# ColinWine/Multi-modal-Multi-label-Facial-Action-Unit-Detection-with-Transformer

Measured on NVIDIA B200. Metric: AVFormer hot-path clips/sec (forward), higher is better.
Workload: dtype bf16

## Files before the change

multi-modal-multi-label-facial-action-unit-detection-with-transformer_b200/csrc/avf_fused_helpers.cuh:

```cuda
#pragma once
#include "avf_common.cuh"

namespace avf {
namespace fused {

#ifdef AVF_FUSED_PROF
static __device__ unsigned long long g_prof[64];
struct Prof {
  long long t0;
  bool on;
  unsigned acc[64];
  __device__ __forceinline__ void start(bool enable) {
    on = enable;
    for (int i = 0; i < 64; ++i) acc[i] = 0;
    t0 = clock64();
  }
  __device__ __forceinline__ void mark(int idx) {
    if (on) {
      const long long t1 = clock64();
      acc[idx] += unsigned(t1 - t0);
      t0 = t1;
    }
  }
  __device__ __forceinline__ void count(int idx) { if (on) acc[idx] += 1; }
  __device__ __forceinline__ void flush(int lo, int hi) {
    if (on) for (int i = lo; i < hi; ++i) g_prof[i] += acc[i];
  }
};
#else
struct Prof {
  __device__ __forceinline__ void start(bool) {}
  __device__ __forceinline__ void mark(int) {}
  __device__ __forceinline__ void count(int) {}
  __device__ __forceinline__ void flush(int, int) {}
};
#endif

__device__ __forceinline__ void bar_sync(int id, int count) { asm volatile("bar.sync %0, %1;" ::"r"(id), "r"(count) : "memory"); }
__device__ __forceinline__ uint32_t cvt_bf16x2(float lo, float hi) {
  uint32_t r;
  asm("cvt.rn.bf16x2.f32 %0, %1, %2;" : "=r"(r) : "f"(hi), "f"(lo));
  return r;
}
__device__ __forceinline__ uint32_t ex2_bf16x2(uint32_t x) {
  uint32_t r;
  asm("ex2.approx.ftz.bf16x2 %0, %1;" : "=r"(r) : "r"(x));
  return r;
}
__device__ __forceinline__ uint32_t tanh_bf16x2(uint32_t x) {
  uint32_t r;
  asm("tanh.approx.bf16x2 %0, %1;" : "=r"(r) : "r"(x));
  return r;
}
__device__ __forceinline__ uint32_t mul_bf16x2(uint32_t a, uint32_t b) {
  uint32_t r;
  asm("mul.rn.bf16x2 %0, %1, %2;" : "=r"(r) : "r"(a), "r"(b));
  return r;
}
__device__ __forceinline__ uint32_t fma_bf16x2(uint32_t a, uint32_t b, uint32_t c) {
  uint32_t r;
  asm("fma.rn.bf16x2 %0, %1, %2, %3;" : "=r"(r) : "r"(a), "r"(b), "r"(c));
  return r;
}
__device__ __forceinline__ uint32_t gelu_bf16x2(uint32_t x) {
  constexpr uint32_t C0 = 0x3F4C3F4Cu;
  constexpr uint32_t C1 = 0x3D123D12u;
  constexpr uint32_t HALF = 0x3F003F00u;
  const uint32_t x2 = mul_bf16x2(x, x);
  const uint32_t u = mul_bf16x2(x, fma_bf16x2(x2, C1, C0));
  const uint32_t hx = mul_bf16x2(x, HALF);
  return fma_bf16x2(hx, tanh_bf16x2(u), hx);
}
__device__ __forceinline__ uint64_t f2_pack(float lo, float hi) {
  uint64_t r;
  asm("mov.b64 %0, {%1, %2};" : "=l"(r) : "f"(lo), "f"(hi));
  return r;
}
__device__ __forceinline__ void f2_unpack(uint64_t v, float& lo, float& hi) { asm("mov.b64 {%0, %1}, %2;" : "=f"(lo), "=f"(hi) : "l"(v)); }
__device__ __forceinline__ uint64_t f2_add(uint64_t a, uint64_t b) {
  uint64_t r;
  asm("add.rn.f32x2 %0, %1, %2;" : "=l"(r) : "l"(a), "l"(b));
  return r;
}
__device__ __forceinline__ uint64_t f2_mul(uint64_t a, uint64_t b) {
  uint64_t r;
  asm("mul.rn.f32x2 %0, %1, %2;" : "=l"(r) : "l"(a), "l"(b));
  return r;
}
__device__ __forceinline__ uint64_t f2_fma(uint64_t a, uint64_t b, uint64_t c) {
  uint64_t r;
  asm("fma.rn.f32x2 %0, %1, %2, %3;" : "=l"(r) : "l"(a), "l"(b), "l"(c));
  return r;
}
__device__ __forceinline__ uint32_t cvt_bf16x2_pair(uint64_t v) {
  float lo, hi;
  f2_unpack(v, lo, hi);
  return cvt_bf16x2(lo, hi);
}

__device__ __forceinline__ void umma_bf16_ts(uint32_t tmem_d, uint32_t tmem_a, uint64_t desc_b, uint32_t idesc, uint32_t acc) {
  asm volatile(
      "{\n\t.reg .pred p;\n\tsetp.ne.b32 p, %4, 0;\n\t"
      "tcgen05.mma.cta_group::1.kind::f16 [%0], [%1], %2, %3, p;\n\t}\n" ::"r"(tmem_d), "r"(tmem_a), "l"(desc_b), "r"(idesc), "r"(acc)
      : "memory");
}
__device__ __forceinline__ void tmem_st4(uint32_t taddr, uint32_t a, uint32_t b, uint32_t c, uint32_t d) {
  asm volatile("tcgen05.st.sync.aligned.32x32b.x4.b32 [%0], {%1, %2, %3, %4};" ::"r"(taddr), "r"(a), "r"(b), "r"(c), "r"(d) : "memory");
}
__device__ __forceinline__ void tmem_st16(uint32_t taddr, const uint32_t (&r)[16]) {
  asm volatile(
      "tcgen05.st.sync.aligned.32x32b.x16.b32 [%0], {%1, %2, %3, %4, %5, %6, %7, %8, %9, %10, %11, %12, %13, %14, %15, %16};" ::"r"(taddr),
      "r"(r[0]), "r"(r[1]), "r"(r[2]), "r"(r[3]), "r"(r[4]), "r"(r[5]), "r"(r[6]), "r"(r[7]), "r"(r[8]), "r"(r[9]), "r"(r[10]), "r"(r[11]),
      "r"(r[12]), "r"(r[13]), "r"(r[14]), "r"(r[15])
      : "memory");
}
__device__ __forceinline__ void tmem_st8(uint32_t taddr, const uint32_t (&r)[8]) {
  asm volatile("tcgen05.st.sync.aligned.32x32b.x8.b32 [%0], {%1, %2, %3, %4, %5, %6, %7, %8};" ::"r"(taddr), "r"(r[0]), "r"(r[1]), "r"(r[2]), "r"(r[3]),
               "r"(r[4]), "r"(r[5]), "r"(r[6]), "r"(r[7])
               : "memory");
}
__device__ __forceinline__ void tmem_st16_zero(uint32_t taddr) {
  asm volatile("tcgen05.st.sync.aligned.32x32b.x16.b32 [%0], {%1, %1, %1, %1, %1, %1, %1, %1, %1, %1, %1, %1, %1, %1, %1, %1};" ::"r"(taddr), "r"(0u)
               : "memory");
}
__device__ __forceinline__ void zero_p_columns(uint32_t taddr, int lo, int hi) {
  int c = lo;
  for (; c + 16 <= hi; c += 16) tmem_st16_zero(taddr + c);
  for (; c + 4 <= hi; c += 4) tmem_st4(taddr + c, 0u, 0u, 0u, 0u);
}
__device__ __forceinline__ void tmem_ld8(uint32_t taddr, uint32_t (&r)[8]) {
  asm volatile("tcgen05.ld.sync.aligned.32x32b.x8.b32 {%0, %1, %2, %3, %4, %5, %6, %7}, [%8];"
               : "=r"(r[0]), "=r"(r[1]), "=r"(r[2]), "=r"(r[3]), "=r"(r[4]), "=r"(r[5]), "=r"(r[6]), "=r"(r[7])
               : "r"(taddr)
               : "memory");
}
__device__ __forceinline__ void bulk_store_1d(void* gdst, const void* smem_src, uint32_t bytes) {
  asm volatile("cp.async.bulk.global.shared::cta.bulk_group [%0], [%1], %2;" ::"l"(reinterpret_cast<uint64_t>(gdst)), "r"(smem_u32(smem_src)),
               "r"(bytes)
               : "memory");
  asm volatile("cp.async.bulk.commit_group;" ::: "memory");
}
__device__ __forceinline__ void bulk_wait_read0() { asm volatile("cp.async.bulk.wait_group.read 0;" ::: "memory"); }
__device__ __forceinline__ void bulk_wait_all0() { asm volatile("cp.async.bulk.wait_group 0;" ::: "memory"); }

__device__ __forceinline__ uint64_t desc_sw64(uint32_t addr) { return make_desc(addr, 16, 512, 4); }

__device__ __forceinline__ uint4 pack8u(const uint32_t* r) {
  uint4 pk;
  pk.x = pack_bf16x2(__uint_as_float(r[0]), __uint_as_float(r[1]));
  pk.y = pack_bf16x2(__uint_as_float(r[2]), __uint_as_float(r[3]));
  pk.z = pack_bf16x2(__uint_as_float(r[4]), __uint_as_float(r[5]));
  pk.w = pack_bf16x2(__uint_as_float(r[6]), __uint_as_float(r[7]));
  return pk;
}

}
}
```

multi-modal-multi-label-facial-action-unit-detection-with-transformer_b200/csrc/avf_layer_fused.cu:

```cuda
#include <cuda.h>

#include "avf_common.cuh"
#include "avf_fused_helpers.cuh"
#include "avf_internal.h"

namespace avf {

int make_tmap_bf16_2d(CUtensorMap* tm, const void* ptr, uint64_t rows, uint64_t cols, uint64_t ld, uint32_t box_rows, uint32_t box_cols = 64);

namespace {
using namespace fused;

constexpr int DIM = 256, HEADS = 8, DH = 32;
constexpr int MAX_DEPTH = 3, MAX_MLP = 1024;
constexpr int NSPLIT = 2;
constexpr int WORKER_T0 = 96;
constexpr int NUM_WORKERS = 128 * NSPLIT;
constexpr int NUM_THREADS = WORKER_T0 + NUM_WORKERS;
constexpr int RING = 9, RING_LO = 2, RING_HI = 4, SLOT_BYTES = 16384;
constexpr int QRING = 6, QSLOT_BYTES = 12288;
template <int D> constexpr int KPH = D / 64;
template <int D> constexpr int NQG = (QRING + KPH<D> - 1) / KPH<D>;
constexpr int MAX_QG = NQG<128>;
static_assert(KPH<256> * (NQG<256> - 1) < QRING && QRING <= KPH<256> * NQG<256>, "head-full barrier parity (D = 256)");
static_assert(KPH<128> * (NQG<128> - 1) < QRING && QRING <= KPH<128> * NQG<128>, "head-full barrier parity (D = 128)");
constexpr int MLPG = 4;
template <int D> constexpr int GSLOTS = MLPG < D / 64 ? MLPG : D / 64;

constexpr int OFF_A0 = 0;
constexpr int OFF_Q = 65536;
constexpr int OFF_K = OFF_Q + 8192;
constexpr int OFF_V = OFF_K + 8192;
constexpr int OFF_RING = OFF_V + 16384;
constexpr int OFF_QRING = OFF_RING + 2 * SLOT_BYTES;
constexpr int OFF_OUTST = OFF_QRING;
static_assert(QRING * QSLOT_BYTES >= 2 * 64 * 256 * 2, "the NCHW output staging lives in the QKV ring");
constexpr int QRING_END = OFF_QRING + QRING * QSLOT_BYTES;
constexpr int OFF_XCH = QRING_END > OFF_Q + RING * SLOT_BYTES ? QRING_END : OFF_Q + RING * SLOT_BYTES;
static_assert(OFF_XCH - OFF_Q >= RING * SLOT_BYTES, "the nine MLP ring slots fit in [OFF_Q, OFF_XCH)");
static_assert(OFF_RING == OFF_Q + RING_LO * SLOT_BYTES, "ring slots are contiguous from OFF_Q");
__host__ __device__ constexpr int slot_offset(uint32_t s) { return OFF_Q + int(s) * SLOT_BYTES; }
constexpr int OFF_VEC = OFF_XCH + 2 * 128 * 4 * 4;
constexpr int V_BOUT = 0, V_BFF2 = DIM, V_BFF1 = 2 * DIM;
constexpr int V_B16 = V_BFF1 + MAX_MLP;
constexpr int OFF_BAR = OFF_VEC + (V_B16 + 512) * 4;
constexpr int SMEM_USED = OFF_BAR + 512;
constexpr int SMEM_ALLOC = SMEM_USED + 1024;
static_assert(SMEM_ALLOC <= 232448, "shared memory budget");

template <int D> constexpr bool A0_HALF = D == 256;
template <int D>
__device__ __forceinline__ constexpr int kpanel(int i) { return A0_HALF<D> ? (((i & 1) << 1) | (i >> 1)) : i; }

constexpr uint32_t TM_X = 0, TM_D1 = 256, TM_O = 352, TM_S = 384, TM_H0 = 256, TM_H1 = 384;

enum {
  B_RING_FULL = 0, B_RING_EMPTY = RING, B_X0_FULL = 2 * RING, B_A0_FREE, B_A0_READY, B_D1_FULL, B_STAGED, B_S_FULL, B_P_READY, B_O_FULL,
  B_O_DRAINED, B_X1_FULL, B_HACC_FULL, B_HACC_FULL1, B_H_READY, B_H_READY1, B_X2_FULL,
  B_QG_FULL, B_QR_EMPTY = B_QG_FULL + MAX_QG, B_A1_FREE = B_QR_EMPTY + QRING, B_OUT_READ, B_QKV_FREE, B_G_FULL, B_TQ_FULL = B_G_FULL + 8, B_A0_HALF = B_TQ_FULL + 4, NUM_BARS
};
static_assert(NUM_BARS * 8 + 8 + 16 <= 512, "barrier block (+ TMEM slot + tile queue)");

__device__ __forceinline__ int* tile_queue(uint64_t* bars) { return reinterpret_cast<int*>(bars + NUM_BARS) + 2; }
__device__ __forceinline__ int next_tile(uint64_t* bars, uint32_t k) {
  mbar_wait(&bars[B_TQ_FULL + (k & 3u)], (k >> 2) & 1u);
  return *reinterpret_cast<volatile int*>(tile_queue(bars) + (k & 3u));
}

enum { IO_NCHW_BF16 = 0, IO_ROWS_F32 = 1 };
constexpr int POS_LD = 64;

enum { PW_INPUT = 0, PW_VEC, PW_LN1, PW_WAIT_D1, PW_E1, PW_WAIT_O, PW_E3, PW_WAIT_S, PW_E2, PW_WAIT_X1, PW_LN2, PW_WAIT_HACC, PW_GELU, PW_WAIT_X2,
       PW_OUTPUT, PW_TILES, PW_E2_LD, PW_E2_EXP, PW_E2_XCH, PW_E2_ST,
       PM_WAIT_A0 = 32, PM_QKV, PM_WAIT_STAGED, PM_S, PM_WAIT_P, PM_PV, PM_WAIT_OD7, PM_OUT, PM_WAIT_A0B, PM_FF1, PM_WAIT_H, PM_FF2, PM_RINGWAIT,
       PM_RW_QKV, PM_RW_OUT, PM_RW_FF1, PM_RW_FF2, PM_REFILL_CYC, PM_REFILL_N };

struct LayerArgs {
  CUtensorMap tm_qkv, tm_out, tm_w1, tm_w2;
  const float *ln1_g, *ln1_b, *b_out, *ln2_g, *ln2_b, *b_ff1, *b_ff2;
  uint64_t pad_;
};

struct FusedArgs {
  LayerArgs layer[MAX_DEPTH];
  const void* in;
  void* out;
  const float* pos;
  const float* w_last;
  float* out21;
  int* decisions;
  const float* pos_t;
  int ld_in, ld_out;
  int* tile_counter;
  int n_seq, n_tok, slot, slot_log2, spt, n_tiles, n_chunks, depth;
};

__device__ unsigned* g_trap_buffer = nullptr;

template <int D>
struct Worker {
  static constexpr int CW = D / NSPLIT;

  uint8_t* smem;
  uint64_t* bars;
  const float* vec;
  uint32_t tl;
  int lane, q, g, row;
  uint32_t xslot;

  __device__ __forceinline__ const float* exchange(float mine) {
    float* s = reinterpret_cast<float*>(smem + OFF_XCH) + xslot * (128 * 4);
    xslot ^= 1;
    s[row * 4 + g] = mine;
    bar_sync(1 + q, 32 * NSPLIT);
    return s + row * 4;
  }
  __device__ __forceinline__ float exchange_sum(float mine) {
    const float* v = exchange(mine);
    return v[0] + v[1];
  }
  __device__ __forceinline__ float exchange_max(float mine) {
    const float* v = exchange(mine);
    return fmaxf(v[0], v[1]);
  }
  __device__ __forceinline__ void arrive(int bar) {
    fence_proxy_async_smem();
    tc_fence_before();
    __syncwarp();
    if (lane == 0) mbar_arrive(&bars[bar]);
  }
  __device__ __forceinline__ void arrive_tmem_only(int bar) {
    tc_fence_before();
    __syncwarp();
    if (lane == 0) mbar_arrive(&bars[bar]);
  }
  struct Stats {
    float shift, s, ss;
    __device__ __forceinline__ void add(const float (&x)[32], bool first) {
      if (first) shift = x[0];
      const uint64_t nshift = f2_pack(-shift, -shift);
      uint64_t s2 = f2_pack(0.f, 0.f), q2 = s2;
#pragma unroll
      for (int j = 0; j < 32; j += 2) {
        const uint64_t d = f2_add(f2_pack(x[j], x[j + 1]), nshift);
        s2 = f2_add(s2, d);
        q2 = f2_fma(d, d, q2);
      }
      float a, b;
      f2_unpack(s2, a, b);
      s += a + b;
      f2_unpack(q2, a, b);
      ss += a + b;
    }
  };
  __device__ __forceinline__ void finish_stats(const Stats& st, float& mean, float& rstd) {
    constexpr float n = float(CW);
    const float mean_g = st.shift + st.s * (1.f / n);
    const float m2_g = fmaxf(st.ss - st.s * st.s * (1.f / n), 0.f);
    mean = exchange_sum(mean_g) * (1.f / NSPLIT);
    const float dm = mean_g - mean;
    const float m2 = exchange_sum(fmaf(dm * dm, n, m2_g));
    rstd = rsqrtf(m2 * (1.f / D) + 1e-5f);
  }
  __device__ __forceinline__ void stats_from_tmem(float& mean, float& rstd) {
    Stats st{0.f, 0.f, 0.f};
#pragma unroll
    for (int c0 = 0; c0 < CW; c0 += 32) {
      float x[32];
      tmem_ld32(tl + TM_X + g * CW + c0, reinterpret_cast<uint32_t(&)[32]>(x));
      tmem_ld_wait();
      st.add(x, c0 == 0);
    }
    finish_stats(st, mean, rstd);
  }
  __device__ __forceinline__ void normalize_from_tmem(float mean, float rstd, int ln_sel, int v_next_bias) {
    const int cbase = g * CW;
    const float nmr = -mean * rstd;
    const uint64_t rstd2 = f2_pack(rstd, rstd), nmr2 = f2_pack(nmr, nmr);
#pragma unroll 1
    for (int c0 = 0; c0 < CW; c0 += 32) {
      float x[32];
      tmem_ld32(tl + TM_X + cbase + c0, reinterpret_cast<uint32_t(&)[32]>(x));
      tmem_ld_wait();
      const int col0 = cbase + c0;
      uint8_t* dst = smem + OFF_A0 + (col0 >> 6) * 16384 + row * 128;
      const int chunk0 = (col0 & 63) >> 3;
#pragma unroll
      for (int ch = 0; ch < 4; ++ch) {
        const __nv_bfloat16* v16 = reinterpret_cast<const __nv_bfloat16*>(vec + V_B16) + ln_sel * (2 * DIM) + col0 + ch * 8;
        const uint4 gm = *reinterpret_cast<const uint4*>(v16), bt = *reinterpret_cast<const uint4*>(v16 + DIM);
        uint4 pk;
        pk.x = fma_bf16x2(cvt_bf16x2_pair(f2_fma(f2_pack(x[ch * 8], x[ch * 8 + 1]), rstd2, nmr2)), gm.x, bt.x);
        pk.y = fma_bf16x2(cvt_bf16x2_pair(f2_fma(f2_pack(x[ch * 8 + 2], x[ch * 8 + 3]), rstd2, nmr2)), gm.y, bt.y);
        pk.z = fma_bf16x2(cvt_bf16x2_pair(f2_fma(f2_pack(x[ch * 8 + 4], x[ch * 8 + 5]), rstd2, nmr2)), gm.z, bt.z);
        pk.w = fma_bf16x2(cvt_bf16x2_pair(f2_fma(f2_pack(x[ch * 8 + 6], x[ch * 8 + 7]), rstd2, nmr2)), gm.w, bt.w);
        *reinterpret_cast<uint4*>(dst + (((chunk0 + ch) ^ (row & 7)) << 4)) = pk;
      }
#pragma unroll
      for (int j = 0; j < 32; j += 4) {
        const ulonglong2 b = *reinterpret_cast<const ulonglong2*>(vec + v_next_bias + col0 + j);
        f2_unpack(f2_add(f2_pack(x[j], x[j + 1]), b.x), x[j], x[j + 1]);
        f2_unpack(f2_add(f2_pack(x[j + 2], x[j + 3]), b.y), x[j + 2], x[j + 3]);
      }
      tmem_st32(tl + TM_X + col0, reinterpret_cast<const uint32_t(&)[32]>(x));
      if (A0_HALF<D> && c0 == 32) arrive(B_A0_HALF);
    }
    tmem_st_wait();
    arrive(B_A0_READY);
  }
};

template <int NC, int TAILV, class W>
__device__ __forceinline__ float softmax_fixed(W& w, uint32_t ts, uint32_t tp, float sm_scale, Prof& pf) {
  float s[NC][8];
#pragma unroll
  for (int c = 0; c < NC; ++c) tmem_ld8(ts + c * 8, reinterpret_cast<uint32_t(&)[8]>(s[c]));
  tmem_ld_wait();
  pf.mark(PW_E2_LD);
  float mc[NC];
#pragma unroll
  for (int c = 0; c < NC; ++c) {
    if (TAILV > 0 && c == NC - 1) {
      mc[c] = s[c][0];
#pragma unroll
      for (int j = 1; j < 8; ++j)
        if (j < TAILV) mc[c] = fmaxf(mc[c], s[c][j]);
    } else {
      mc[c] = fmaxf(fmaxf(fmaxf(s[c][0], s[c][1]), fmaxf(s[c][2], s[c][3])), fmaxf(fmaxf(s[c][4], s[c][5]), fmaxf(s[c][6], s[c][7])));
    }
  }
  float mloc = mc[0];
#pragma unroll
  for (int c = 1; c < NC; ++c) mloc = fmaxf(mloc, mc[c]);
  pf.mark(PW_E2_EXP);
  const float mrow = w.exchange_max(mloc);
  pf.mark(PW_E2_XCH);
  const float nml = -mrow * sm_scale;
  const uint64_t sc2 = f2_pack(sm_scale, sm_scale), nml2 = f2_pack(nml, nml);
  uint64_t sum2 = f2_pack(0.f, 0.f);
  float sum_lo = 0.f;
#pragma unroll
  for (int c = 0; c < NC; ++c) {
    const int nv = (TAILV > 0 && c == NC - 1) ? TAILV : 8;
    uint32_t e[4];
#pragma unroll
    for (int j = 0; j < 4; ++j) {
      if (2 * j + 1 < nv) {
        e[j] = ex2_bf16x2(cvt_bf16x2_pair(f2_fma(f2_pack(s[c][2 * j], s[c][2 * j + 1]), sc2, nml2)));
        sum2 = f2_add(sum2, f2_pack(__uint_as_float(e[j] << 16), __uint_as_float(e[j] & 0xFFFF0000u)));
      } else if (2 * j < nv) {
        e[j] = ex2_bf16x2(cvt_bf16x2(fmaf(s[c][2 * j], sm_scale, nml), -INFINITY)) & 0xFFFFu;
        sum_lo += __uint_as_float(e[j] << 16);
      } else {
        e[j] = 0u;
      }
    }
    tmem_st4(tp + c * 4, e[0], e[1], e[2], e[3]);
  }
  float a, b;
  f2_unpack(sum2, a, b);
  return sum_lo + (a + b);
}

__host__ __device__ constexpr int slot_of(int n_tok) { return n_tok <= 16 ? 16 : (n_tok <= 32 ? 32 : 64); }
__host__ __device__ constexpr int log2_of(int v) { return v == 16 ? 4 : (v == 32 ? 5 : 6); }

template <int IO, int NTOK, int D>
__device__ void worker_main(const FusedArgs& a, uint8_t* smem, uint64_t* bars, uint32_t tmem) {
  using W = Worker<D>;
  constexpr int CW = W::CW;
  W w;
  w.smem = smem;
  w.bars = bars;
  w.vec = reinterpret_cast<const float*>(smem + OFF_VEC);
  const int wt = threadIdx.x - WORKER_T0;
  w.lane = wt & 31;
  w.q = (threadIdx.x >> 5) & 3;
  w.g = wt >> 7;
  w.row = w.q * 32 + w.lane;
  w.tl = tmem + (uint32_t(w.q * 32) << 16);
  w.xslot = 0;
  const int q = w.q, g = w.g, row = w.row;
  const uint32_t tl = w.tl;
  const float* vec = w.vec;
  const int n_tok = NTOK ? NTOK : a.n_tok, slot = NTOK ? slot_of(NTOK) : a.slot, spt = NTOK ? 128 / slot_of(NTOK) : a.spt;
  const int slot_log2 = NTOK ? log2_of(slot_of(NTOK)) : a.slot_log2;
  const int seq_in_tile = row >> slot_log2, t_in_seq = row & (slot - 1);
  const int lo = seq_in_tile * slot, hi = lo + n_tok;
  const int s0 = (q * 32) >> slot_log2, s1 = (q * 32 + 31) >> slot_log2;
  const int c_lo = (s0 * slot) >> 3, c_hi = (s1 * slot + n_tok + 7) >> 3;
  constexpr int MAXC = 8 / NSPLIT;
  const int per = (c_hi - c_lo + NSPLIT - 1) / NSPLIT;
  const int my_c0 = c_lo + g * per;
  const int my_nc = max(0, min(per, c_hi - my_c0));
  const bool warp_one_seq = s0 == s1;
  const float sm_scale = 1.4426950408889634f * rsqrtf(float(DH));
  uint32_t n_x0 = 0, n_x1 = 0, n_x2 = 0, n_hacc0 = 0, n_hacc1 = 0;
  bool vec_loaded = false;
  Prof pf;
  pf.start(blockIdx.x == 0 && wt == 0);

  for (uint32_t tk = 0;; ++tk) {
    const int tile = next_tile(bars, tk);
    if (tile < 0) break;
    const int seqs_here = min(spt, a.n_seq - tile * spt);
    const bool valid = seq_in_tile < seqs_here && t_in_seq < n_tok;
    const size_t grow = (size_t(tile) * spt + seq_in_tile) * n_tok + t_in_seq;

    float mean, rstd;
    {
      typename W::Stats st{0.f, 0.f, 0.f};
      const int t_safe = valid ? t_in_seq : 0, seq_safe = valid ? seq_in_tile : 0;
      const float* pp = (IO == IO_ROWS_F32 && a.pos != nullptr) ? a.pos + t_safe * D + g * CW : nullptr;
      const float4* ppt = reinterpret_cast<const float4*>(a.pos_t) + size_t(g * CW / 4) * POS_LD + t_safe;
      if constexpr (IO == IO_NCHW_BF16) mbar_wait(&bars[B_X0_FULL], (n_x0++) & 1);
      const __nv_bfloat16* src16 = reinterpret_cast<const __nv_bfloat16*>(smem + OFF_A0) + size_t(seq_safe * D + g * CW) * n_tok + t_safe;
      const float* src32 = static_cast<const float*>(a.in) + ((size_t(tile) * spt + seq_safe) * n_tok + t_safe) * a.ld_in + g * CW;
#pragma unroll 1
      for (int c0 = 0; c0 < CW; c0 += 32) {
        float x[32];
        if constexpr (IO == IO_NCHW_BF16) {
          float4 p[8];
#pragma unroll
          for (int j = 0; j < 8; ++j) p[j] = __ldg(ppt + (c0 / 4 + j) * POS_LD);
#pragma unroll
          for (int j = 0; j < 8; ++j) {
            f2_unpack(f2_add(f2_pack(__bfloat162float(src16[(c0 + 4 * j) * n_tok]), __bfloat162float(src16[(c0 + 4 * j + 1) * n_tok])),
                             f2_pack(p[j].x, p[j].y)), x[4 * j], x[4 * j + 1]);
            f2_unpack(f2_add(f2_pack(__bfloat162float(src16[(c0 + 4 * j + 2) * n_tok]), __bfloat162float(src16[(c0 + 4 * j + 3) * n_tok])),
                             f2_pack(p[j].z, p[j].w)), x[4 * j + 2], x[4 * j + 3]);
          }
        } else {
          float4 p4[8];
          if (pp != nullptr) {
#pragma unroll
            for (int j = 0; j < 8; ++j) p4[j] = __ldg(reinterpret_cast<const float4*>(pp + c0) + j);
          }
#pragma unroll
          for (int j = 0; j < 32; j += 4) {
            const float4 x4 = *reinterpret_cast<const float4*>(src32 + c0 + j);
            x[j] = x4.x; x[j + 1] = x4.y; x[j + 2] = x4.z; x[j + 3] = x4.w;
          }
          if (pp != nullptr) {
#pragma unroll
            for (int j = 0; j < 8; ++j) {
              x[4 * j] += p4[j].x; x[4 * j + 1] += p4[j].y; x[4 * j + 2] += p4[j].z; x[4 * j + 3] += p4[j].w;
            }
          }
        }
        st.add(x, c0 == 0);
        tmem_st32(tl + TM_X + g * CW + c0, reinterpret_cast<const uint32_t(&)[32]>(x));
      }
      tmem_st_wait();
      w.finish_stats(st, mean, rstd);
      if constexpr (IO == IO_NCHW_BF16) {
        if (threadIdx.x == WORKER_T0) {
          bulk_wait_read0();
          mbar_arrive(&bars[B_OUT_READ]);
        }
        bar_sync(5, NUM_WORKERS);
      }
    }
    pf.mark(PW_INPUT);

    for (int l = 0; l < a.depth; ++l) {
      const LayerArgs& L = a.layer[l];
      if (a.depth > 1 || !vec_loaded) {
        if (vec_loaded) bar_sync(5, NUM_WORKERS);
        float* vs = reinterpret_cast<float*>(smem + OFF_VEC);
        for (int i = wt; i < D; i += NUM_WORKERS) {
          vs[V_BOUT + i] = L.b_out[i]; vs[V_BFF2 + i] = L.b_ff2[i];
          __nv_bfloat16* v16 = reinterpret_cast<__nv_bfloat16*>(vs + V_B16);
          v16[i] = __float2bfloat16_rn(L.ln1_g[i]); v16[DIM + i] = __float2bfloat16_rn(L.ln1_b[i]);
          v16[2 * DIM + i] = __float2bfloat16_rn(L.ln2_g[i]); v16[3 * DIM + i] = __float2bfloat16_rn(L.ln2_b[i]);
        }
        for (int i = wt; i < a.n_chunks * 128; i += NUM_WORKERS) vs[V_BFF1 + i] = L.b_ff1[i];
        bar_sync(5, NUM_WORKERS);
        vec_loaded = true;
      }
      pf.mark(PW_VEC);
      w.normalize_from_tmem(mean, rstd, 0, V_BOUT);
      pf.mark(PW_LN1);

      float inv_l = 0.f;
#pragma unroll 1
      for (int h = 0; h <= HEADS; ++h) {
        if (h < HEADS) {
          mbar_wait(&bars[B_D1_FULL], h & 1);
          tc_fence_after();
          pf.mark(PW_WAIT_D1);
          constexpr int NCH = 12 / NSPLIT;
          const uint32_t sw = uint32_t((row >> 1) & 3);
          uint32_t r[NCH * 8];
          tmem_ld32(tl + TM_D1 + g * 48, reinterpret_cast<uint32_t(&)[32]>(r[0]));
          tmem_ld16(tl + TM_D1 + g * 48 + 32, reinterpret_cast<uint32_t(&)[16]>(r[32]));
          tmem_ld_wait();
#pragma unroll
          for (int c = 0; c < NCH; ++c) {
            const int id = g * NCH + c;
            uint8_t* base = id < 4 ? smem + OFF_Q : (id < 8 ? smem + OFF_K : smem + OFF_V + (h & 1) * 8192);
            *reinterpret_cast<uint4*>(base + row * 64 + ((uint32_t(id & 3) ^ sw) << 4)) = pack8u(&r[c * 8]);
          }
          w.arrive(B_STAGED);
          pf.mark(PW_E1);
        }
        if (h > 0) {
          mbar_wait(&bars[B_O_FULL], (h - 1) & 1);
          tc_fence_after();
          pf.mark(PW_WAIT_O);
          constexpr int OW = DH / NSPLIT;
          uint32_t r[OW];
          tmem_ld16(tl + TM_O + g * OW, reinterpret_cast<uint32_t(&)[16]>(r[0]));
          tmem_ld_wait();
          {
            const float* sums = reinterpret_cast<const float*>(smem + OFF_XCH) + ((h - 1) & 1) * (128 * 4) + row * 4 + 2;
            asm("rcp.approx.ftz.f32 %0, %1;" : "=f"(inv_l) : "f"(sums[0] + sums[1]));
          }
          const uint64_t inv2 = f2_pack(inv_l, inv_l);
          uint32_t pk[8];
#pragma unroll
          for (int j = 0; j < 8; ++j) pk[j] = cvt_bf16x2_pair(f2_mul(f2_pack(__uint_as_float(r[2 * j]), __uint_as_float(r[2 * j + 1])), inv2));
          tmem_st8(tl + TM_O + g * OW, pk);
          tmem_st_wait();
          w.arrive_tmem_only(B_O_DRAINED);
          pf.mark(PW_E3);
        }
        if (h < HEADS) {
          mbar_wait(&bars[B_S_FULL], h & 1);
          tc_fence_after();
          pf.mark(PW_WAIT_S);
          if constexpr (NTOK > 32) {
            constexpr int NCH_ALL = (NTOK + 7) / 8, NC1 = NCH_ALL - 4, TAILV = NTOK & 7;
            static_assert(NC1 >= 1 && NC1 <= 4, "softmax split");
            const uint32_t sb = tl + TM_S + uint32_t(seq_in_tile) * 64, pb = tl + TM_S + uint32_t(seq_in_tile) * 32;
            const float sum_g = g == 0 ? softmax_fixed<4, 0>(w, sb, pb, sm_scale, pf) : softmax_fixed<NC1, TAILV>(w, sb + 32, pb + 16, sm_scale, pf);
            reinterpret_cast<float*>(smem + OFF_XCH)[(h & 1) * (128 * 4) + row * 4 + 2 + g] = sum_g;
            if (g == seq_in_tile) {
              zero_p_columns(tl + TM_S, 32 * g + NCH_ALL * 4, 32 * g + 32);
            } else {
              tmem_st16_zero(tl + TM_S + 32 * g);
              tmem_st16_zero(tl + TM_S + 32 * g + 16);
            }
            tmem_st_wait();
            pf.mark(PW_E2_ST);
            w.arrive_tmem_only(B_P_READY);
            pf.mark(PW_E2);
          } else {
          float s[MAXC][8];
#pragma unroll
          for (int c = 0; c < MAXC; ++c)
            if (c < my_nc) tmem_ld8(tl + TM_S + (my_c0 + c) * 8, reinterpret_cast<uint32_t(&)[8]>(s[c]));
          tmem_ld_wait();
          pf.mark(PW_E2_LD);
          float mloc = -INFINITY;
#pragma unroll
          for (int c = 0; c < MAXC; ++c) {
            if (c < my_nc) {
              const int col0 = (my_c0 + c) * 8;
              if (!warp_one_seq || col0 + 8 > hi) {
#pragma unroll
                for (int j = 0; j < 8; ++j) s[c][j] = (col0 + j >= lo && col0 + j < hi) ? s[c][j] : -INFINITY;
              }
              mloc = fmaxf(mloc, fmaxf(fmaxf(fmaxf(s[c][0], s[c][1]), fmaxf(s[c][2], s[c][3])), fmaxf(fmaxf(s[c][4], s[c][5]), fmaxf(s[c][6], s[c][7]))));
            }
          }
          pf.mark(PW_E2_EXP);
          const float mrow = w.exchange_max(mloc);
          pf.mark(PW_E2_XCH);
          const float nml = -mrow * sm_scale;
          float sum_g = 0.f;
#pragma unroll
          for (int c = 0; c < MAXC; ++c) {
            if (c < my_nc) {
              uint32_t e[4];
#pragma unroll
              for (int j = 0; j < 4; ++j) {
                e[j] = ex2_bf16x2(cvt_bf16x2(fmaf(s[c][2 * j], sm_scale, nml), fmaf(s[c][2 * j + 1], sm_scale, nml)));
                sum_g += __uint_as_float(e[j] << 16) + __uint_as_float(e[j] & 0xFFFF0000u);
              }
              tmem_st4(tl + TM_S + (my_c0 + c) * 4, e[0], e[1], e[2], e[3]);
            }
          }
          reinterpret_cast<float*>(smem + OFF_XCH)[(h & 1) * (128 * 4) + row * 4 + 2 + g] = sum_g;
          {
            const int z_lo = g * 32, z_hi = z_lo + 32, w_lo = c_lo * 4, w_hi = c_hi * 4;
            zero_p_columns(tl + TM_S, z_lo, min(z_hi, max(z_lo, w_lo)));
            zero_p_columns(tl + TM_S, max(z_lo, min(z_hi, w_hi)), z_hi);
          }
          tmem_st_wait();
          pf.mark(PW_E2_ST);
          w.arrive_tmem_only(B_P_READY);
          pf.mark(PW_E2);
          }
        }
      }

      mbar_wait(&bars[B_X1_FULL], (n_x1++) & 1);
      tc_fence_after();
      pf.mark(PW_WAIT_X1);
      w.stats_from_tmem(mean, rstd);
      w.normalize_from_tmem(mean, rstd, 1, V_BFF2);
      pf.mark(PW_LN2);

#pragma unroll 1
      for (int c = 0; c < a.n_chunks; ++c) {
        const int b = c & 1;
        if (b == 0) mbar_wait(&bars[B_HACC_FULL], (n_hacc0++) & 1);
        else mbar_wait(&bars[B_HACC_FULL1], (n_hacc1++) & 1);
        tc_fence_after();
        pf.mark(PW_WAIT_HACC);
        constexpr int HW = 128 / NSPLIT;
        const uint32_t hbase = tl + (b ? TM_H1 : TM_H0) + g * HW;
#pragma unroll
        for (int c0 = 0; c0 < HW; c0 += 32) {
          const float* bias = vec + V_BFF1 + c * 128 + g * HW + c0;
          uint32_t r[32], yk[16];
          tmem_ld32(hbase + c0, r);
          tmem_ld_wait();
#pragma unroll
          for (int j = 0; j < 32; j += 4) {
            const float4 b4 = *reinterpret_cast<const float4*>(bias + j);
            yk[j / 2] = gelu_bf16x2(cvt_bf16x2_pair(f2_add(f2_pack(__uint_as_float(r[j]), __uint_as_float(r[j + 1])), f2_pack(b4.x, b4.y))));
            yk[j / 2 + 1] = gelu_bf16x2(cvt_bf16x2_pair(f2_add(f2_pack(__uint_as_float(r[j + 2]), __uint_as_float(r[j + 3])), f2_pack(b4.z, b4.w))));
          }
          tmem_st16(hbase + c0 / 2, yk);
        }
        tmem_st_wait();
        w.arrive_tmem_only(B_H_READY + b);
        pf.mark(PW_GELU);
      }

      mbar_wait(&bars[B_X2_FULL], (n_x2++) & 1);
      tc_fence_after();
      pf.mark(PW_WAIT_X2);
      if (l + 1 < a.depth) w.stats_from_tmem(mean, rstd);
    }

    {
      __nv_bfloat16* dst16 = reinterpret_cast<__nv_bfloat16*>(smem + OFF_OUTST) + size_t(seq_in_tile * D + g * CW) * n_tok + t_in_seq;
      const bool store = valid && (IO == IO_NCHW_BF16 || a.out != nullptr);
      float* dst32 = static_cast<float*>(a.out) + grow * a.ld_out + g * CW;
      const bool logits = IO == IO_ROWS_F32 && a.w_last != nullptr;
      const float* wl = logits ? a.w_last + (valid ? t_in_seq : 0) * D + g * CW : nullptr;
      float dot = 0.f;
#pragma unroll 1
      for (int c0 = 0; c0 < CW; c0 += 32) {
        float x[32];
        tmem_ld32(tl + TM_X + g * CW + c0, reinterpret_cast<uint32_t(&)[32]>(x));
        tmem_ld_wait();
        if (store) {
          if constexpr (IO == IO_NCHW_BF16) {
#pragma unroll
            for (int j = 0; j < 32; ++j) dst16[(c0 + j) * n_tok] = __float2bfloat16_rn(x[j]);
          } else {
#pragma unroll
            for (int j = 0; j < 32; j += 4) *reinterpret_cast<float4*>(dst32 + c0 + j) = make_float4(x[j], x[j + 1], x[j + 2], x[j + 3]);
          }
        }
        if constexpr (IO == IO_ROWS_F32) {
          if (logits) {
#pragma unroll
            for (int j = 0; j < 32; j += 4) {
              const float4 w4 = __ldg(reinterpret_cast<const float4*>(wl + c0 + j));
              dot = fmaf(x[j], w4.x, fmaf(x[j + 1], w4.y, fmaf(x[j + 2], w4.z, fmaf(x[j + 3], w4.w, dot))));
            }
          }
        }
      }
      if constexpr (IO == IO_ROWS_F32) {
        if (logits) {
          const float lg = w.exchange_sum(dot);
          const size_t clip = grow / 12;
          if (valid && g == 0) {
            if (a.out21 != nullptr) a.out21[clip * 21 + t_in_seq] = lg;
            if (a.decisions != nullptr) a.decisions[clip * 12 + t_in_seq] = lg > 0.f ? 1 : 0;
          }
          if (valid && g == 1 && t_in_seq < 9 && a.out21 != nullptr) a.out21[clip * 21 + 12 + t_in_seq] = 0.f;
        }
      }
      if constexpr (IO == IO_NCHW_BF16) {
        fence_proxy_async_smem();
        bar_sync(5, NUM_WORKERS);
        if (threadIdx.x == WORKER_T0) {
          __nv_bfloat16* gdst = static_cast<__nv_bfloat16*>(a.out) + size_t(tile) * spt * n_tok * D;
          bulk_store_1d(gdst, smem + OFF_OUTST, uint32_t(seqs_here) * n_tok * D * 2);
        }
      }
    }
    pf.mark(PW_OUTPUT);
    pf.count(PW_TILES);
  }
  pf.flush(0, 32);
  if constexpr (IO == IO_NCHW_BF16) {
    if (threadIdx.x == WORKER_T0) bulk_wait_all0();
  }
}

template <int IO, int D>
__device__ void producer_main(const FusedArgs& a, uint8_t* smem, uint64_t* bars) {
  uint32_t it = 0;
  int load_tile = blockIdx.x;
  uint32_t n_free = 0;
  bool need_free = false;
  auto poll_loader = [&]() {
    if (IO != IO_NCHW_BF16 || load_tile < 0) return;
    if (need_free) {
      if (!mbar_test_wait(&bars[B_A0_FREE], n_free & 1)) return;
      ++n_free;
    }
    const int seqs_here = min(a.spt, a.n_seq - load_tile * a.spt);
    const uint32_t bytes = uint32_t(seqs_here) * a.n_tok * D * 2;
    mbar_expect_tx(&bars[B_X0_FULL], bytes);
    bulk_load_1d(smem + OFF_A0, static_cast<const __nv_bfloat16*>(a.in) + size_t(load_tile) * a.spt * a.n_tok * D, bytes, &bars[B_X0_FULL]);
    load_tile = -1;
    need_free = true;
  };
  uint32_t pbits = 0, n_gate = 0;
  auto poll_wait = [&](uint64_t* bar, uint32_t parity) {
    if (mbar_try_wait(bar, parity)) return;
    poll_loader();
    const long long t0 = clock64();
    while (!mbar_try_wait(bar, parity)) {
      poll_loader();
      if (clock64() - t0 > 4000000000LL) {
        unsigned* tb = g_trap_buffer;
        if (tb != nullptr) {
          tb[0] = blockIdx.x; tb[1] = threadIdx.x; tb[2] = (smem_u32(bar) & 1023u) >> 3; tb[3] = parity;
          __threadfence_system();
        }
        printf("avf: fused encoder producer timed out (block %d item %u)\n", blockIdx.x, it);
        __trap();
      }
    }
  };
  uint32_t gidx = 0;
  auto load = [&](uint32_t s, const CUtensorMap* tm, int c0, int c1, uint64_t* full_bar, uint32_t expect_bytes) {
    poll_wait(&bars[B_RING_EMPTY + s], ((pbits >> s) & 1u) ^ 1u);
    pbits ^= 1u << s;
    if (expect_bytes != 0) mbar_expect_tx(full_bar, expect_bytes);
    tma_load_2d(smem + slot_offset(s), tm, full_bar, c0, c1);
    ++it;
  };
  uint32_t kpub = 0;
  auto publish = [&](int t) {
    tile_queue(bars)[kpub & 3u] = t;
    mbar_arrive(&bars[B_TQ_FULL + (kpub & 3u)]);
    ++kpub;
  };
  int cur = blockIdx.x;
  publish(cur);
  for (;;) {
    int nxt;
    if (a.tile_counter != nullptr) nxt = atomicAdd(a.tile_counter, 1) + int(gridDim.x);
    else nxt = cur + int(gridDim.x);
    if (nxt >= a.n_tiles) nxt = -1;
    publish(nxt);
    if (IO == IO_NCHW_BF16) {
      while (load_tile >= 0) poll_loader();
      load_tile = nxt;
    }
    for (int l = 0; l < a.depth; ++l) {
      const LayerArgs& L = a.layer[l];
      for (int h = 0; h < HEADS; ++h) {
        const uint32_t s = RING_LO + h % (RING_HI - RING_LO);
        load(s, &L.tm_out, h * DH, 0, &bars[B_RING_FULL + s], D * DH * 2);
      }
      poll_wait(&bars[B_QKV_FREE], (n_gate++) & 1);
      uint32_t m = 0;
      constexpr int G = GSLOTS<D>, NH = D / 128;
      auto ff1 = [&](int c) {
        for (int kp = 0; kp < D / 64; ++kp) {
          if (kp % G == 0) ++gidx;
          load((m++) % RING, &L.tm_w1, kpanel<D>(kp) * 64, c * 128, &bars[B_G_FULL + ((gidx - 1) & 7u)], kp % G == 0 ? G * SLOT_BYTES : 0);
        }
      };
      auto ff2 = [&](int c) {
        for (int i = 0; i < 2 * NH; ++i) {
          const int kp = i / NH, nh = i % NH;
          if (i % G == 0) ++gidx;
          load((m++) % RING, &L.tm_w2, c * 128 + kp * 64, nh * 128, &bars[B_G_FULL + ((gidx - 1) & 7u)], i % G == 0 ? G * SLOT_BYTES : 0);
        }
      };
      ff1(0);
      if (a.n_chunks > 1) ff1(1);
      for (int c = 0; c < a.n_chunks; ++c) {
        ff2(c);
        if (c + 2 < a.n_chunks) ff1(c + 2);
      }
    }
    if (nxt < 0) break;
    cur = nxt;
  }
}

template <int IO, int D>
__device__ void qkv_producer_main(const FusedArgs& a, uint8_t* smem, uint64_t* bars) {
  uint32_t qit = 0, hq = 0, n_free = 0, n_read = 0;
  bool first = true;
  for (uint32_t tk = 0; next_tile(bars, tk) >= 0; ++tk) {
    if constexpr (IO == IO_NCHW_BF16) mbar_wait(&bars[B_OUT_READ], (n_read++) & 1);
    for (int l = 0; l < a.depth; ++l) {
      const LayerArgs& L = a.layer[l];
      if (!first) mbar_wait(&bars[B_A1_FREE], (n_free++) & 1);
      first = false;
      for (int h = 0; h < HEADS; ++h, ++hq) {
        uint64_t* fb = &bars[B_QG_FULL + (hq % uint32_t(NQG<D>))];
        for (int kp = 0; kp < KPH<D>; ++kp) {
          const uint32_t s = qit % QRING, ph = (qit / QRING) & 1;
          mbar_wait(&bars[B_QR_EMPTY + s], ph ^ 1);
          uint8_t* d = smem + OFF_QRING + s * QSLOT_BYTES;
          if (kp == 0) mbar_expect_tx(fb, KPH<D> * QSLOT_BYTES);
          for (int s3 = 0; s3 < 3; ++s3) tma_load_2d(d + s3 * 4096, &L.tm_qkv, fb, kpanel<D>(kp) * 64, s3 * (HEADS * DH) + h * DH);
          ++qit;
        }
      }
    }
  }
}

template <int D>
__device__ void mma_main(const FusedArgs& a, uint8_t* smem, uint64_t* bars, uint32_t tmem) {
  const bool leader = elect_one();
  const uint32_t a0 = smem_u32(smem + OFF_A0);
  const uint32_t qs = smem_u32(smem + OFF_Q), ks = smem_u32(smem + OFF_K), vs = smem_u32(smem + OFF_V);
  const uint32_t smem0 = smem_u32(smem), qring = smem_u32(smem + OFF_QRING);
  const int kmax = 128;
  const uint32_t id_qkv = make_idesc_bf16(128, 96), id_s = make_idesc_bf16(128, kmax), id_pv = make_idesc_bf16(128, DH, 0, 1),
                 id_128 = make_idesc_bf16(128, 128), id_out = make_idesc_bf16(128, D);
  uint32_t obits = 0, m = 0, qit = 0, hq = 0, gidx = 0, n_a0 = 0, n_hready[2] = {0, 0};
  Prof pf;
  pf.start(blockIdx.x == 0 && leader);
  int ring_phase = PM_QKV;
  auto slot_wait = [&](uint32_t s) -> uint32_t {
    pf.mark(ring_phase);
    mbar_wait(&bars[B_RING_FULL + s], (obits >> s) & 1u);
    obits ^= 1u << s;
    tc_fence_after();
    pf.mark(PM_RW_OUT);
    return smem0 + uint32_t(slot_offset(s));
  };
  auto group_wait = [&]() {
    pf.mark(ring_phase);
    mbar_wait(&bars[B_G_FULL + (gidx & 7u)], (gidx >> 3) & 1u);
    ++gidx;
    tc_fence_after();
    pf.mark(ring_phase == PM_FF1 ? PM_RW_FF1 : PM_RW_FF2);
  };
  auto slot_release = [&](uint32_t s) {
    if (leader) umma_commit(&bars[B_RING_EMPTY + s]);
  };
  auto a0_wait = [&](int i, bool fresh) {
    if constexpr (A0_HALF<D>) {
      if (!fresh || (i != 0 && i != 2)) return;
      pf.mark(ring_phase);
      if (i == 0) mbar_wait(&bars[B_A0_HALF], n_a0 & 1);
      else mbar_wait(&bars[B_A0_READY], (n_a0++) & 1);
    } else {
      if (!fresh || i != 0) return;
      pf.mark(ring_phase);
      mbar_wait(&bars[B_A0_READY], (n_a0++) & 1);
    }
    tc_fence_after();
    pf.mark(ring_phase == PM_QKV ? PM_WAIT_A0 : PM_WAIT_A0B);
  };
  auto qkv = [&](bool fresh) {
    pf.mark(ring_phase);
    mbar_wait(&bars[B_QG_FULL + (hq % uint32_t(NQG<D>))], (hq / uint32_t(NQG<D>)) & 1u);
    ++hq;
    tc_fence_after();
    pf.mark(PM_RW_QKV);
    for (int i = 0; i < KPH<D>; ++i) {
      const int kp = kpanel<D>(i);
      a0_wait(i, fresh);
      const uint32_t s = qit % QRING;
      const uint64_t da = make_desc_sw128_kmajor(a0 + kp * 16384), db = make_desc_sw128_kmajor(qring + s * QSLOT_BYTES);
#pragma unroll
      for (int k = 0; k < 4; ++k) if (leader) umma_bf16(tmem + TM_D1, da + uint64_t(k * 2), db + uint64_t(k * 2), id_qkv, (i | k) != 0 ? 1u : 0u);
      if (leader) umma_commit(&bars[B_QR_EMPTY + s]);
      ++qit;
    }
    if (leader) umma_commit(&bars[B_D1_FULL]);
  };
  auto outproj = [&](int h) {
    const uint32_t s = RING_LO + h % (RING_HI - RING_LO), sb = slot_wait(s);
    const uint64_t db = desc_sw64(sb);
    if (leader) umma_bf16_ts(tmem + TM_X, tmem + TM_O, db, id_out, 1u);
    if (leader) umma_bf16_ts(tmem + TM_X, tmem + TM_O + 16, db + 2, id_out, 1u);
    slot_release(s);
  };
  bool last_layer = false;
  auto ff1 = [&](int c, bool fresh) {
    const uint32_t d = tmem + ((c & 1) ? TM_H1 : TM_H0);
    for (int i = 0; i < D / 64; ++i) {
      const int kp = kpanel<D>(i);
      if (i % GSLOTS<D> == 0) group_wait();
      a0_wait(i, fresh);
      const uint32_t s = (m++) % RING, sb = smem0 + uint32_t(slot_offset(s));
      const uint64_t da = make_desc_sw128_kmajor(a0 + kp * 16384), db = make_desc_sw128_kmajor(sb);
#pragma unroll
      for (int k = 0; k < 4; ++k) if (leader) umma_bf16(d, da + uint64_t(k * 2), db + uint64_t(k * 2), id_128, (i | k) != 0 ? 1u : 0u);
      slot_release(s);
    }
    if (leader) umma_commit(&bars[B_HACC_FULL + (c & 1)]);
    if (c == a.n_chunks - 1 && last_layer) if (leader) umma_commit(&bars[B_A0_FREE]);
  };

  for (uint32_t tk = 0; next_tile(bars, tk) >= 0; ++tk) {
    for (int l = 0; l < a.depth; ++l) {
      last_layer = l == a.depth - 1;
      ring_phase = PM_QKV;
      qkv(true);
      pf.mark(PM_QKV);
      for (int h = 0; h < HEADS; ++h) {
        mbar_wait(&bars[B_STAGED], h & 1);
        tc_fence_after();
        pf.mark(PM_WAIT_STAGED);
        {
          const uint64_t da = desc_sw64(qs), db = desc_sw64(ks);
          if (leader) umma_bf16(tmem + TM_S, da, db, id_s, 0u);
          if (leader) umma_bf16(tmem + TM_S, da + 2, db + 2, id_s, 1u);
          if (leader) umma_commit(&bars[B_S_FULL]);
        }
        pf.mark(PM_S);
        if (h + 1 < HEADS) qkv(false);
        pf.mark(PM_QKV);
        if (h > 0) {
          mbar_wait(&bars[B_O_DRAINED], (h - 1) & 1);
          tc_fence_after();
          pf.mark(PM_WAIT_OD7);
          ring_phase = PM_OUT;
          outproj(h - 1);
          pf.mark(PM_OUT);
          ring_phase = PM_QKV;
        }
        mbar_wait(&bars[B_P_READY], h & 1);
        tc_fence_after();
        pf.mark(PM_WAIT_P);
        for (int k = 0; k < kmax / 16; ++k)
          if (leader) umma_bf16_ts(tmem + TM_O, tmem + TM_S + uint32_t(k * 8), desc_sw64(vs + (h & 1) * 8192 + k * 1024), id_pv, k != 0 ? 1u : 0u);
        if (leader) umma_commit(&bars[B_O_FULL]);
        pf.mark(PM_PV);
      }
      mbar_wait(&bars[B_O_DRAINED], (HEADS - 1) & 1);
      tc_fence_after();
      pf.mark(PM_WAIT_OD7);
      ring_phase = PM_OUT;
      outproj(HEADS - 1);
      if (leader) umma_commit(&bars[B_X1_FULL]);
      if (leader) umma_commit(&bars[B_QKV_FREE]);
      m = 0;
      pf.mark(PM_OUT);

      ring_phase = PM_FF1;
      ff1(0, true);
      if (a.n_chunks > 1) ff1(1, false);
      for (int c = 0; c < a.n_chunks; ++c) {
        const int b = c & 1;
        pf.mark(PM_FF1);
        mbar_wait(&bars[B_H_READY + b], (n_hready[b]++) & 1);
        tc_fence_after();
        pf.mark(PM_WAIT_H);
        ring_phase = PM_FF2;
        for (int kp = 0; kp < 2; ++kp)
          for (int nh = 0; nh < D / 128; ++nh) {
            if ((kp * (D / 128) + nh) % GSLOTS<D> == 0) group_wait();
            const uint32_t s = (m++) % RING, sb = smem0 + uint32_t(slot_offset(s));
            const uint32_t ta = tmem + (b ? TM_H1 : TM_H0) + uint32_t(kp * 64);
            const uint64_t db = make_desc_sw128_kmajor(sb);
#pragma unroll
            for (int k = 0; k < 4; ++k) if (leader) umma_bf16_ts(tmem + TM_X + nh * 128, ta + uint32_t(k * 8), db + uint64_t(k * 2), id_128, 1u);
            slot_release(s);
          }
        pf.mark(PM_FF2);
        ring_phase = PM_FF1;
        if (c + 2 < a.n_chunks) ff1(c + 2, false);
      }
      if (leader) umma_commit(&bars[B_X2_FULL]);
      if (leader) umma_commit(&bars[B_A1_FREE]);
    }
  }
  pf.flush(32, 64);
}

template <int IO, int NTOK, int D>
__global__ void __launch_bounds__(NUM_THREADS, 1) encoder_fused_kernel(const __grid_constant__ FusedArgs a) {
  extern __shared__ __align__(1024) uint8_t smem_raw[];
  uint8_t* smem = smem_raw;
  if (threadIdx.x == 0 && (smem_u32(smem_raw) & 1023u) != 0u) {
    printf("avf: encoder_fused_kernel: dynamic shared memory base is not 1024-byte aligned enough\n");
    __trap();
  }
  uint64_t* bars = reinterpret_cast<uint64_t*>(smem + OFF_BAR);
  uint32_t* tmem_slot = reinterpret_cast<uint32_t*>(bars + NUM_BARS);
  const int warp = threadIdx.x >> 5, lane = threadIdx.x & 31;

  if (threadIdx.x == 0) {
    for (int l = 0; l < a.depth; ++l) {
      tma_prefetch_desc(&a.layer[l].tm_qkv);
      tma_prefetch_desc(&a.layer[l].tm_out);
      tma_prefetch_desc(&a.layer[l].tm_w1);
      tma_prefetch_desc(&a.layer[l].tm_w2);
    }
    for (int i = 0; i < NUM_BARS; ++i) {
      const bool by_workers = i == B_A0_READY || i == B_A0_HALF || i == B_STAGED || i == B_P_READY || i == B_O_DRAINED || i == B_H_READY || i == B_H_READY1;
      mbar_init(&bars[i], by_workers ? NUM_WORKERS / 32 : 1);
    }
    fence_barrier_init();
  }
  if (warp == 1) {
    tmem_alloc(tmem_slot, 512);
    tmem_relinquish();
  }
  tc_fence_before();
  __syncthreads();
  tc_fence_after();
  const uint32_t tmem = *tmem_slot;
  pdl_wait();
  pdl_trigger();

  if (warp == 0) {
    if (lane == 0) producer_main<IO, D>(a, smem, bars);
  } else if (warp == 1) {
    mma_main<D>(a, smem, bars, tmem);
  } else if (warp == 2) {
    if (lane == 0) qkv_producer_main<IO, D>(a, smem, bars);
  } else {
    worker_main<IO, NTOK, D>(a, smem, bars, tmem);
  }

  tc_fence_before();
  __syncthreads();
  if (warp == 1) tmem_dealloc(tmem, 512);
}

__global__ void __launch_bounds__(256) pos_transpose_kernel(const float* __restrict__ pos, float* __restrict__ pos_t, int n_tok, int* tile_counter) {
  pdl_wait();
  pdl_trigger();
  if (blockIdx.x == 0 && threadIdx.x == 0 && tile_counter != nullptr) *tile_counter = 0;
  const int c = blockIdx.x * 4 + (threadIdx.x & 3), t = threadIdx.x >> 2;
  pos_t[(blockIdx.x * POS_LD + t) * 4 + (threadIdx.x & 3)] = t < n_tok ? pos[t * DIM + c] : 0.f;
}

int sm_count_cached() { return sm_count_of_current_device(); }

}

int fused_set_trap_buffer(void* host_mapped_words) {
  unsigned* p = static_cast<unsigned*>(host_mapped_words);
  AVF_CUDA(cudaMemcpyToSymbol(g_trap_buffer, &p, sizeof(p)));
  return 0;
}

int fused_prof_read(unsigned long long* out64, int reset) {
#ifdef AVF_FUSED_PROF
  AVF_CUDA(cudaDeviceSynchronize());
  AVF_CUDA(cudaMemcpyFromSymbol(out64, g_prof, sizeof(unsigned long long) * 64));
  if (reset) {
    static unsigned long long zeros[64] = {0};
    AVF_CUDA(cudaMemcpyToSymbol(g_prof, zeros, sizeof(zeros)));
  }
  return 0;
#else
  (void)out64; (void)reset;
  return AVF_EUNSUPPORTED;
#endif
}

bool encoder_fused_supported(const avf_stack_shape* s) {
  return (s->dim == 256 || s->dim == 128) && s->heads == HEADS && s->dim_head == DH && s->mlp_dim % 128 == 0 && s->mlp_dim >= 128 && s->mlp_dim <= MAX_MLP && s->n_tok >= 1 &&
         s->n_tok <= 64 && s->depth >= 1 && s->depth <= MAX_DEPTH;
}

size_t encoder_fused_scratch_bytes() { return size_t(DIM) * POS_LD * sizeof(float) + 64; }

int encoder_fused(int io_kind, const avf_stack_shape* s, const avf_layer_weights* L, const void* in, int ld_in, void* out, int ld_out,
                  const float* pos, void* scratch, const float* w_last, float* out21, int* decisions, cudaStream_t st) {
  AVF_REQUIRE(encoder_fused_supported(s), AVF_EUNSUPPORTED, "fused encoder: unsupported shape dim=%d heads=%d dh=%d mlp=%d n_tok=%d depth=%d",
              s->dim, s->heads, s->dim_head, s->mlp_dim, s->n_tok, s->depth);
  AVF_REQUIRE(io_kind == IO_ROWS_F32 || (pos != nullptr && scratch != nullptr), AVF_EINVAL,
              "fused encoder: NCHW input needs the positional embedding and the scratch buffer");
  AVF_REQUIRE(io_kind == IO_ROWS_F32 || s->dim == DIM, AVF_EUNSUPPORTED, "fused encoder: the NCHW form is dim %d only", DIM);
  AVF_REQUIRE(io_kind == IO_NCHW_BF16 || (ld_in % 4 == 0 && (out == nullptr || ld_out % 4 == 0)), AVF_EINVAL, "fused encoder: row strides must be multiples of 4");
  AVF_REQUIRE(w_last == nullptr || (io_kind == IO_ROWS_F32 && s->n_tok == 12), AVF_EINVAL, "fused encoder: AU logits need 12-token rows");
  AVF_REQUIRE(out != nullptr || w_last != nullptr, AVF_EINVAL, "fused encoder: no output");
  static thread_local FusedArgs a;
  static_assert(sizeof(FusedArgs) <= 4000, "kernel parameter space");
  a.in = in; a.out = out; a.pos = pos; a.pos_t = static_cast<const float*>(scratch); a.ld_in = ld_in; a.ld_out = ld_out;
  a.w_last = w_last; a.out21 = out21; a.decisions = decisions;
  a.tile_counter = nullptr;
  if (io_kind == IO_NCHW_BF16) {
    a.tile_counter = reinterpret_cast<int*>(static_cast<uint8_t*>(scratch) + size_t(DIM) * POS_LD * sizeof(float));
    launch_pdl(pos_transpose_kernel, DIM / 4, 256, 0, st, pos, static_cast<float*>(scratch), s->n_tok, a.tile_counter);
    AVF_LAUNCH_CHECK("pos_transpose_kernel");
  }
  a.n_seq = s->n_seq; a.n_tok = s->n_tok;
  a.slot = 16; a.slot_log2 = 4;
  while (a.slot < s->n_tok) { a.slot *= 2; ++a.slot_log2; }
  a.spt = 128 / a.slot;
  a.n_tiles = ceil_div(s->n_seq, a.spt);
  a.n_chunks = s->mlp_dim / 128; a.depth = s->depth;
  const int inner = HEADS * DH, D = s->dim;
  for (int l = 0; l < s->depth; ++l) {
    LayerArgs& A = a.layer[l];
    int e;
    if ((e = make_tmap_bf16_2d(&A.tm_qkv, L[l].w_qkv, 3 * inner, D, D, 32))) return e;
    if ((e = make_tmap_bf16_2d(&A.tm_out, L[l].w_out, D, inner, inner, D, DH))) return e;
    if ((e = make_tmap_bf16_2d(&A.tm_w1, L[l].w_ff1, s->mlp_dim, D, D, 128))) return e;
    if ((e = make_tmap_bf16_2d(&A.tm_w2, L[l].w_ff2, D, s->mlp_dim, s->mlp_dim, 128))) return e;
    A.ln1_g = L[l].ln1_gamma; A.ln1_b = L[l].ln1_beta; A.b_out = L[l].b_out;
    A.ln2_g = L[l].ln2_gamma; A.ln2_b = L[l].ln2_beta; A.b_ff1 = L[l].b_ff1; A.b_ff2 = L[l].b_ff2;
  }
  static PerDeviceOnce once;
  if (once.first()) {
    AVF_CUDA(cudaFuncSetAttribute(encoder_fused_kernel<IO_NCHW_BF16, 49, 256>, cudaFuncAttributeMaxDynamicSharedMemorySize, SMEM_ALLOC));
    AVF_CUDA(cudaFuncSetAttribute(encoder_fused_kernel<IO_NCHW_BF16, 0, 256>, cudaFuncAttributeMaxDynamicSharedMemorySize, SMEM_ALLOC));
    AVF_CUDA(cudaFuncSetAttribute(encoder_fused_kernel<IO_ROWS_F32, 0, 256>, cudaFuncAttributeMaxDynamicSharedMemorySize, SMEM_ALLOC));
    AVF_CUDA(cudaFuncSetAttribute(encoder_fused_kernel<IO_ROWS_F32, 0, 128>, cudaFuncAttributeMaxDynamicSharedMemorySize, SMEM_ALLOC));
  }
  const int cap = sm_cap();
  const int grid = min(a.n_tiles, cap > 0 ? min(cap, sm_count_cached()) : sm_count_cached());
  if (io_kind == IO_NCHW_BF16 && a.n_tok == 49)
    launch_pdl(encoder_fused_kernel<IO_NCHW_BF16, 49, 256>, grid, NUM_THREADS, SMEM_ALLOC, st, a);
  else if (io_kind == IO_NCHW_BF16)
    launch_pdl(encoder_fused_kernel<IO_NCHW_BF16, 0, 256>, grid, NUM_THREADS, SMEM_ALLOC, st, a);
  else if (D == 256)
    launch_pdl(encoder_fused_kernel<IO_ROWS_F32, 0, 256>, grid, NUM_THREADS, SMEM_ALLOC, st, a);
  else
    launch_pdl(encoder_fused_kernel<IO_ROWS_F32, 0, 128>, grid, NUM_THREADS, SMEM_ALLOC, st, a);
  AVF_LAUNCH_CHECK("encoder_fused_kernel");
  return 0;
}

}
```

Baseline: 490,400.

## Ping-pong TMEM residual buffers with a dedicated drain warpgroup for NCHW output

For the NCHW bf16 path, the residual stream X alternates between two TMEM halves per tile, and scratch (D1/O/S/H) uses the other half. A new 128-thread drain warpgroup writes out the finished tile's output while workers and the MMA warp start on the next tile, replacing the inline output store through the QKV ring. setmaxnreg moves registers from the small roles to the workers. Barrier waits also gain a timeout trap. The cost is added barrier complexity, a tighter TMEM layout, and a larger thread count.

```diff
diff --git a/multi-modal-multi-label-facial-action-unit-detection-with-transformer_b200/csrc/avf_fused_helpers.cuh b/multi-modal-multi-label-facial-action-unit-detection-with-transformer_b200/csrc/avf_fused_helpers.cuh
--- a/multi-modal-multi-label-facial-action-unit-detection-with-transformer_b200/csrc/avf_fused_helpers.cuh
+++ b/multi-modal-multi-label-facial-action-unit-detection-with-transformer_b200/csrc/avf_fused_helpers.cuh
@@ -134,14 +134,10 @@
                : "r"(taddr)
                : "memory");
 }
-__device__ __forceinline__ void bulk_store_1d(void* gdst, const void* smem_src, uint32_t bytes) {
-  asm volatile("cp.async.bulk.global.shared::cta.bulk_group [%0], [%1], %2;" ::"l"(reinterpret_cast<uint64_t>(gdst)), "r"(smem_u32(smem_src)),
-               "r"(bytes)
-               : "memory");
-  asm volatile("cp.async.bulk.commit_group;" ::: "memory");
+
+__device__ __forceinline__ void bulk_prefetch_l2(const void* gsrc, uint32_t bytes) {
+  asm volatile("cp.async.bulk.prefetch.L2.global [%0], %1;" ::"l"(reinterpret_cast<uint64_t>(gsrc)), "r"(bytes) : "memory");
 }
-__device__ __forceinline__ void bulk_wait_read0() { asm volatile("cp.async.bulk.wait_group.read 0;" ::: "memory"); }
-__device__ __forceinline__ void bulk_wait_all0() { asm volatile("cp.async.bulk.wait_group 0;" ::: "memory"); }
 
 __device__ __forceinline__ uint64_t desc_sw64(uint32_t addr) { return make_desc(addr, 16, 512, 4); }
 
diff --git a/multi-modal-multi-label-facial-action-unit-detection-with-transformer_b200/csrc/avf_layer_fused.cu b/multi-modal-multi-label-facial-action-unit-detection-with-transformer_b200/csrc/avf_layer_fused.cu
--- a/multi-modal-multi-label-facial-action-unit-detection-with-transformer_b200/csrc/avf_layer_fused.cu
+++ b/multi-modal-multi-label-facial-action-unit-detection-with-transformer_b200/csrc/avf_layer_fused.cu
@@ -14,9 +14,13 @@
 constexpr int DIM = 256, HEADS = 8, DH = 32;
 constexpr int MAX_DEPTH = 3, MAX_MLP = 1024;
 constexpr int NSPLIT = 2;
-constexpr int WORKER_T0 = 96;
 constexpr int NUM_WORKERS = 128 * NSPLIT;
-constexpr int NUM_THREADS = WORKER_T0 + NUM_WORKERS;
+enum { IO_NCHW_BF16 = 0, IO_ROWS_F32 = 1 };
+template <int IO> constexpr bool PINGPONG = IO == IO_NCHW_BF16;
+template <int IO> constexpr int WORKER_T0 = PINGPONG<IO> ? 128 : 96;
+template <int IO> constexpr int NUM_THREADS = WORKER_T0<IO> + NUM_WORKERS + (PINGPONG<IO> ? 128 : 0);
+constexpr int REG_SMALL = 56, REG_WORKER = 200;
+static_assert(2 * REG_SMALL + 2 * REG_WORKER == 4 * 65536 / NUM_THREADS<IO_NCHW_BF16>, "setmaxnreg shares = the launch pool");
 constexpr int RING = 9, RING_LO = 2, RING_HI = 4, SLOT_BYTES = 16384;
 constexpr int QRING = 6, QSLOT_BYTES = 12288;
 template <int D> constexpr int KPH = D / 64;
@@ -33,8 +37,6 @@
 constexpr int OFF_V = OFF_K + 8192;
 constexpr int OFF_RING = OFF_V + 16384;
 constexpr int OFF_QRING = OFF_RING + 2 * SLOT_BYTES;
-constexpr int OFF_OUTST = OFF_QRING;
-static_assert(QRING * QSLOT_BYTES >= 2 * 64 * 256 * 2, "the NCHW output staging lives in the QKV ring");
 constexpr int QRING_END = OFF_QRING + QRING * QSLOT_BYTES;
 constexpr int OFF_XCH = QRING_END > OFF_Q + RING * SLOT_BYTES ? QRING_END : OFF_Q + RING * SLOT_BYTES;
 static_assert(OFF_XCH - OFF_Q >= RING * SLOT_BYTES, "the nine MLP ring slots fit in [OFF_Q, OFF_XCH)");
@@ -52,28 +54,47 @@
 template <int D>
 __device__ __forceinline__ constexpr int kpanel(int i) { return A0_HALF<D> ? (((i & 1) << 1) | (i >> 1)) : i; }
 
-constexpr uint32_t TM_X = 0, TM_D1 = 256, TM_O = 352, TM_S = 384, TM_H0 = 256, TM_H1 = 384;
+constexpr uint32_t TM_D1 = 0, TM_O = 96, TM_S = 128, TM_H0 = 0, TM_H1 = 128;
+template <int IO>
+struct TileTmem {
+  uint32_t x, s;
+  __device__ __forceinline__ explicit TileTmem(uint32_t tk) : x(PINGPONG<IO> ? (tk & 1u) * 256u : 0u), s(256u - x) {}
+};
 
 enum {
   B_RING_FULL = 0, B_RING_EMPTY = RING, B_X0_FULL = 2 * RING, B_A0_FREE, B_A0_READY, B_D1_FULL, B_STAGED, B_S_FULL, B_P_READY, B_O_FULL,
   B_O_DRAINED, B_X1_FULL, B_HACC_FULL, B_HACC_FULL1, B_H_READY, B_H_READY1, B_X2_FULL,
-  B_QG_FULL, B_QR_EMPTY = B_QG_FULL + MAX_QG, B_A1_FREE = B_QR_EMPTY + QRING, B_OUT_READ, B_QKV_FREE, B_G_FULL, B_TQ_FULL = B_G_FULL + 8, B_A0_HALF = B_TQ_FULL + 4, NUM_BARS
+  B_QG_FULL, B_QR_EMPTY = B_QG_FULL + MAX_QG, B_A1_FREE = B_QR_EMPTY + QRING, B_X_DONE, B_DRAINED, B_QKV_FREE, B_G_FULL, B_TQ_FULL = B_G_FULL + 8, B_A0_HALF = B_TQ_FULL + 4, NUM_BARS
 };
 static_assert(NUM_BARS * 8 + 8 + 16 <= 512, "barrier block (+ TMEM slot + tile queue)");
 
+__device__ unsigned* g_trap_buffer = nullptr;
+__device__ __forceinline__ void trap_timed_out(uint64_t* bar, uint32_t parity) {
+  unsigned* tb = g_trap_buffer;
+  if (tb != nullptr) {
+    tb[0] = blockIdx.x; tb[1] = threadIdx.x; tb[2] = (smem_u32(bar) & 1023u) >> 3; tb[3] = parity;
+    __threadfence_system();
+  }
+  __trap();
+}
+__device__ __forceinline__ void bar_wait(uint64_t* bar, uint32_t parity) {
+  if (mbar_try_wait(bar, parity)) return;
+  const long long t0 = clock64();
+  while (!mbar_try_wait_sleep(bar, parity))
+    if (clock64() - t0 > 4000000000LL) trap_timed_out(bar, parity);
+}
 __device__ __forceinline__ int* tile_queue(uint64_t* bars) { return reinterpret_cast<int*>(bars + NUM_BARS) + 2; }
 __device__ __forceinline__ int next_tile(uint64_t* bars, uint32_t k) {
-  mbar_wait(&bars[B_TQ_FULL + (k & 3u)], (k >> 2) & 1u);
+  bar_wait(&bars[B_TQ_FULL + (k & 3u)], (k >> 2) & 1u);
   return *reinterpret_cast<volatile int*>(tile_queue(bars) + (k & 3u));
 }
 
-enum { IO_NCHW_BF16 = 0, IO_ROWS_F32 = 1 };
 constexpr int POS_LD = 64;
 
 enum { PW_INPUT = 0, PW_VEC, PW_LN1, PW_WAIT_D1, PW_E1, PW_WAIT_O, PW_E3, PW_WAIT_S, PW_E2, PW_WAIT_X1, PW_LN2, PW_WAIT_HACC, PW_GELU, PW_WAIT_X2,
-       PW_OUTPUT, PW_TILES, PW_E2_LD, PW_E2_EXP, PW_E2_XCH, PW_E2_ST,
+       PW_OUTPUT, PW_TILES, PW_E2_LD, PW_E2_EXP, PW_E2_XCH, PW_E2_ST, PW_WAIT_X0,
        PM_WAIT_A0 = 32, PM_QKV, PM_WAIT_STAGED, PM_S, PM_WAIT_P, PM_PV, PM_WAIT_OD7, PM_OUT, PM_WAIT_A0B, PM_FF1, PM_WAIT_H, PM_FF2, PM_RINGWAIT,
-       PM_RW_QKV, PM_RW_OUT, PM_RW_FF1, PM_RW_FF2, PM_REFILL_CYC, PM_REFILL_N };
+       PM_RW_QKV, PM_RW_OUT, PM_RW_FF1, PM_RW_FF2, PM_WAIT_DRAIN };
 
 struct LayerArgs {
   CUtensorMap tm_qkv, tm_out, tm_w1, tm_w2;
@@ -95,8 +116,6 @@
   int n_seq, n_tok, slot, slot_log2, spt, n_tiles, n_chunks, depth;
 };
 
-__device__ unsigned* g_trap_buffer = nullptr;
-
 template <int D>
 struct Worker {
   static constexpr int CW = D / NSPLIT;
@@ -105,6 +124,7 @@
   uint64_t* bars;
   const float* vec;
   uint32_t tl;
+  uint32_t tx;
   int lane, q, g, row;
   uint32_t xslot;
 
@@ -167,7 +187,7 @@
 #pragma unroll
     for (int c0 = 0; c0 < CW; c0 += 32) {
       float x[32];
-      tmem_ld32(tl + TM_X + g * CW + c0, reinterpret_cast<uint32_t(&)[32]>(x));
+      tmem_ld32(tx + g * CW + c0, reinterpret_cast<uint32_t(&)[32]>(x));
       tmem_ld_wait();
       st.add(x, c0 == 0);
     }
@@ -180,7 +200,7 @@
 #pragma unroll 1
     for (int c0 = 0; c0 < CW; c0 += 32) {
       float x[32];
-      tmem_ld32(tl + TM_X + cbase + c0, reinterpret_cast<uint32_t(&)[32]>(x));
+      tmem_ld32(tx + cbase + c0, reinterpret_cast<uint32_t(&)[32]>(x));
       tmem_ld_wait();
       const int col0 = cbase + c0;
       uint8_t* dst = smem + OFF_A0 + (col0 >> 6) * 16384 + row * 128;
@@ -202,7 +222,7 @@
         f2_unpack(f2_add(f2_pack(x[j], x[j + 1]), b.x), x[j], x[j + 1]);
         f2_unpack(f2_add(f2_pack(x[j + 2], x[j + 3]), b.y), x[j + 2], x[j + 3]);
       }
-      tmem_st32(tl + TM_X + col0, reinterpret_cast<const uint32_t(&)[32]>(x));
+      tmem_st32(tx + col0, reinterpret_cast<const uint32_t(&)[32]>(x));
       if (A0_HALF<D> && c0 == 32) arrive(B_A0_HALF);
     }
     tmem_st_wait();
@@ -273,7 +293,7 @@
   w.smem = smem;
   w.bars = bars;
   w.vec = reinterpret_cast<const float*>(smem + OFF_VEC);
-  const int wt = threadIdx.x - WORKER_T0;
+  const int wt = threadIdx.x - WORKER_T0<IO>;
   w.lane = wt & 31;
   w.q = (threadIdx.x >> 5) & 3;
   w.g = wt >> 7;
@@ -303,6 +323,9 @@
   for (uint32_t tk = 0;; ++tk) {
     const int tile = next_tile(bars, tk);
     if (tile < 0) break;
+    const TileTmem<IO> tm(tk);
+    w.tx = tl + tm.x;
+    const uint32_t ts = tl + tm.s;
     const int seqs_here = min(spt, a.n_seq - tile * spt);
     const bool valid = seq_in_tile < seqs_here && t_in_seq < n_tok;
     const size_t grow = (size_t(tile) * spt + seq_in_tile) * n_tok + t_in_seq;
@@ -313,7 +336,10 @@
       const int t_safe = valid ? t_in_seq : 0, seq_safe = valid ? seq_in_tile : 0;
       const float* pp = (IO == IO_ROWS_F32 && a.pos != nullptr) ? a.pos + t_safe * D + g * CW : nullptr;
       const float4* ppt = reinterpret_cast<const float4*>(a.pos_t) + size_t(g * CW / 4) * POS_LD + t_safe;
-      if constexpr (IO == IO_NCHW_BF16) mbar_wait(&bars[B_X0_FULL], (n_x0++) & 1);
+      if constexpr (IO == IO_NCHW_BF16) {
+        bar_wait(&bars[B_X0_FULL], (n_x0++) & 1);
+        pf.mark(PW_WAIT_X0);
+      }
       const __nv_bfloat16* src16 = reinterpret_cast<const __nv_bfloat16*>(smem + OFF_A0) + size_t(seq_safe * D + g * CW) * n_tok + t_safe;
       const float* src32 = static_cast<const float*>(a.in) + ((size_t(tile) * spt + seq_safe) * n_tok + t_safe) * a.ld_in + g * CW;
 #pragma unroll 1
@@ -349,17 +375,11 @@
           }
         }
         st.add(x, c0 == 0);
-        tmem_st32(tl + TM_X + g * CW + c0, reinterpret_cast<const uint32_t(&)[32]>(x));
+        tmem_st32(w.tx + g * CW + c0, reinterpret_cast<const uint32_t(&)[32]>(x));
       }
       tmem_st_wait();
       w.finish_stats(st, mean, rstd);
-      if constexpr (IO == IO_NCHW_BF16) {
-        if (threadIdx.x == WORKER_T0) {
-          bulk_wait_read0();
-          mbar_arrive(&bars[B_OUT_READ]);
-        }
-        bar_sync(5, NUM_WORKERS);
-      }
+      if constexpr (IO == IO_NCHW_BF16) bar_sync(5, NUM_WORKERS);
     }
     pf.mark(PW_INPUT);
 
@@ -386,14 +406,14 @@
 #pragma unroll 1
       for (int h = 0; h <= HEADS; ++h) {
         if (h < HEADS) {
-          mbar_wait(&bars[B_D1_FULL], h & 1);
+          bar_wait(&bars[B_D1_FULL], h & 1);
           tc_fence_after();
           pf.mark(PW_WAIT_D1);
           constexpr int NCH = 12 / NSPLIT;
           const uint32_t sw = uint32_t((row >> 1) & 3);
           uint32_t r[NCH * 8];
-          tmem_ld32(tl + TM_D1 + g * 48, reinterpret_cast<uint32_t(&)[32]>(r[0]));
-          tmem_ld16(tl + TM_D1 + g * 48 + 32, reinterpret_cast<uint32_t(&)[16]>(r[32]));
+          tmem_ld32(ts + TM_D1 + g * 48, reinterpret_cast<uint32_t(&)[32]>(r[0]));
+          tmem_ld16(ts + TM_D1 + g * 48 + 32, reinterpret_cast<uint32_t(&)[16]>(r[32]));
           tmem_ld_wait();
 #pragma unroll
           for (int c = 0; c < NCH; ++c) {
@@ -405,12 +425,12 @@
           pf.mark(PW_E1);
         }
         if (h > 0) {
-          mbar_wait(&bars[B_O_FULL], (h - 1) & 1);
+          bar_wait(&bars[B_O_FULL], (h - 1) & 1);
           tc_fence_after();
           pf.mark(PW_WAIT_O);
           constexpr int OW = DH / NSPLIT;
           uint32_t r[OW];
-          tmem_ld16(tl + TM_O + g * OW, reinterpret_cast<uint32_t(&)[16]>(r[0]));
+          tmem_ld16(ts + TM_O + g * OW, reinterpret_cast<uint32_t(&)[16]>(r[0]));
           tmem_ld_wait();
           {
             const float* sums = reinterpret_cast<const float*>(smem + OFF_XCH) + ((h - 1) & 1) * (128 * 4) + row * 4 + 2;
@@ -420,26 +440,26 @@
           uint32_t pk[8];
 #pragma unroll
           for (int j = 0; j < 8; ++j) pk[j] = cvt_bf16x2_pair(f2_mul(f2_pack(__uint_as_float(r[2 * j]), __uint_as_float(r[2 * j + 1])), inv2));
-          tmem_st8(tl + TM_O + g * OW, pk);
+          tmem_st8(ts + TM_O + g * OW, pk);
           tmem_st_wait();
           w.arrive_tmem_only(B_O_DRAINED);
           pf.mark(PW_E3);
         }
         if (h < HEADS) {
-          mbar_wait(&bars[B_S_FULL], h & 1);
+          bar_wait(&bars[B_S_FULL], h & 1);
           tc_fence_after();
           pf.mark(PW_WAIT_S);
           if constexpr (NTOK > 32) {
             constexpr int NCH_ALL = (NTOK + 7) / 8, NC1 = NCH_ALL - 4, TAILV = NTOK & 7;
             static_assert(NC1 >= 1 && NC1 <= 4, "softmax split");
-            const uint32_t sb = tl + TM_S + uint32_t(seq_in_tile) * 64, pb = tl + TM_S + uint32_t(seq_in_tile) * 32;
+            const uint32_t sb = ts + TM_S + uint32_t(seq_in_tile) * 64, pb = ts + TM_S + uint32_t(seq_in_tile) * 32;
             const float sum_g = g == 0 ? softmax_fixed<4, 0>(w, sb, pb, sm_scale, pf) : softmax_fixed<NC1, TAILV>(w, sb + 32, pb + 16, sm_scale, pf);
             reinterpret_cast<float*>(smem + OFF_XCH)[(h & 1) * (128 * 4) + row * 4 + 2 + g] = sum_g;
             if (g == seq_in_tile) {
-              zero_p_columns(tl + TM_S, 32 * g + NCH_ALL * 4, 32 * g + 32);
+              zero_p_columns(ts + TM_S, 32 * g + NCH_ALL * 4, 32 * g + 32);
             } else {
-              tmem_st16_zero(tl + TM_S + 32 * g);
-              tmem_st16_zero(tl + TM_S + 32 * g + 16);
+              tmem_st16_zero(ts + TM_S + 32 * g);
+              tmem_st16_zero(ts + TM_S + 32 * g + 16);
             }
             tmem_st_wait();
             pf.mark(PW_E2_ST);
@@ -449,7 +469,7 @@
           float s[MAXC][8];
 #pragma unroll
           for (int c = 0; c < MAXC; ++c)
-            if (c < my_nc) tmem_ld8(tl + TM_S + (my_c0 + c) * 8, reinterpret_cast<uint32_t(&)[8]>(s[c]));
+            if (c < my_nc) tmem_ld8(ts + TM_S + (my_c0 + c) * 8, reinterpret_cast<uint32_t(&)[8]>(s[c]));
           tmem_ld_wait();
           pf.mark(PW_E2_LD);
           float mloc = -INFINITY;
@@ -478,14 +498,14 @@
                 e[j] = ex2_bf16x2(cvt_bf16x2(fmaf(s[c][2 * j], sm_scale, nml), fmaf(s[c][2 * j + 1], sm_scale, nml)));
                 sum_g += __uint_as_float(e[j] << 16) + __uint_as_float(e[j] & 0xFFFF0000u);
               }
-              tmem_st4(tl + TM_S + (my_c0 + c) * 4, e[0], e[1], e[2], e[3]);
+              tmem_st4(ts + TM_S + (my_c0 + c) * 4, e[0], e[1], e[2], e[3]);
             }
           }
           reinterpret_cast<float*>(smem + OFF_XCH)[(h & 1) * (128 * 4) + row * 4 + 2 + g] = sum_g;
           {
             const int z_lo = g * 32, z_hi = z_lo + 32, w_lo = c_lo * 4, w_hi = c_hi * 4;
-            zero_p_columns(tl + TM_S, z_lo, min(z_hi, max(z_lo, w_lo)));
-            zero_p_columns(tl + TM_S, max(z_lo, min(z_hi, w_hi)), z_hi);
+            zero_p_columns(ts + TM_S, z_lo, min(z_hi, max(z_lo, w_lo)));
+            zero_p_columns(ts + TM_S, max(z_lo, min(z_hi, w_hi)), z_hi);
           }
           tmem_st_wait();
           pf.mark(PW_E2_ST);
@@ -495,7 +515,7 @@
         }
       }
 
-      mbar_wait(&bars[B_X1_FULL], (n_x1++) & 1);
+      bar_wait(&bars[B_X1_FULL], (n_x1++) & 1);
       tc_fence_after();
       pf.mark(PW_WAIT_X1);
       w.stats_from_tmem(mean, rstd);
@@ -505,12 +525,12 @@
 #pragma unroll 1
       for (int c = 0; c < a.n_chunks; ++c) {
         const int b = c & 1;
-        if (b == 0) mbar_wait(&bars[B_HACC_FULL], (n_hacc0++) & 1);
-        else mbar_wait(&bars[B_HACC_FULL1], (n_hacc1++) & 1);
+        if (b == 0) bar_wait(&bars[B_HACC_FULL], (n_hacc0++) & 1);
+        else bar_wait(&bars[B_HACC_FULL1], (n_hacc1++) & 1);
         tc_fence_after();
         pf.mark(PW_WAIT_HACC);
         constexpr int HW = 128 / NSPLIT;
-        const uint32_t hbase = tl + (b ? TM_H1 : TM_H0) + g * HW;
+        const uint32_t hbase = ts + (b ? TM_H1 : TM_H0) + g * HW;
 #pragma unroll
         for (int c0 = 0; c0 < HW; c0 += 32) {
           const float* bias = vec + V_BFF1 + c * 128 + g * HW + c0;
@@ -530,75 +550,86 @@
         pf.mark(PW_GELU);
       }
 
-      mbar_wait(&bars[B_X2_FULL], (n_x2++) & 1);
+      bar_wait(&bars[B_X2_FULL], (n_x2++) & 1);
       tc_fence_after();
       pf.mark(PW_WAIT_X2);
       if (l + 1 < a.depth) w.stats_from_tmem(mean, rstd);
     }
 
-    {
-      __nv_bfloat16* dst16 = reinterpret_cast<__nv_bfloat16*>(smem + OFF_OUTST) + size_t(seq_in_tile * D + g * CW) * n_tok + t_in_seq;
-      const bool store = valid && (IO == IO_NCHW_BF16 || a.out != nullptr);
+    if constexpr (IO == IO_ROWS_F32) {
+      const bool store = valid && a.out != nullptr;
       float* dst32 = static_cast<float*>(a.out) + grow * a.ld_out + g * CW;
-      const bool logits = IO == IO_ROWS_F32 && a.w_last != nullptr;
+      const bool logits = a.w_last != nullptr;
       const float* wl = logits ? a.w_last + (valid ? t_in_seq : 0) * D + g * CW : nullptr;
       float dot = 0.f;
 #pragma unroll 1
       for (int c0 = 0; c0 < CW; c0 += 32) {
         float x[32];
-        tmem_ld32(tl + TM_X + g * CW + c0, reinterpret_cast<uint32_t(&)[32]>(x));
+        tmem_ld32(w.tx + g * CW + c0, reinterpret_cast<uint32_t(&)[32]>(x));
         tmem_ld_wait();
         if (store) {
-          if constexpr (IO == IO_NCHW_BF16) {
-#pragma unroll
-            for (int j = 0; j < 32; ++j) dst16[(c0 + j) * n_tok] = __float2bfloat16_rn(x[j]);
-          } else {
-#pragma unroll
-            for (int j = 0; j < 32; j += 4) *reinterpret_cast<float4*>(dst32 + c0 + j) = make_float4(x[j], x[j + 1], x[j + 2], x[j + 3]);
-          }
-        }
-        if constexpr (IO == IO_ROWS_F32) {
-          if (logits) {
-#pragma unroll
-            for (int j = 0; j < 32; j += 4) {
-              const float4 w4 = __ldg(reinterpret_cast<const float4*>(wl + c0 + j));
-              dot = fmaf(x[j], w4.x, fmaf(x[j + 1], w4.y, fmaf(x[j + 2], w4.z, fmaf(x[j + 3], w4.w, dot))));
-            }
-          }
-        }
-      }
-      if constexpr (IO == IO_ROWS_F32) {
+#pragma unroll
+          for (int j = 0; j < 32; j += 4) *reinterpret_cast<float4*>(dst32 + c0 + j) = make_float4(x[j], x[j + 1], x[j + 2], x[j + 3]);
+        }
         if (logits) {
-          const float lg = w.exchange_sum(dot);
-          const size_t clip = grow / 12;
-          if (valid && g == 0) {
-            if (a.out21 != nullptr) a.out21[clip * 21 + t_in_seq] = lg;
-            if (a.decisions != nullptr) a.decisions[clip * 12 + t_in_seq] = lg > 0.f ? 1 : 0;
-          }
-          if (valid && g == 1 && t_in_seq < 9 && a.out21 != nullptr) a.out21[clip * 21 + 12 + t_in_seq] = 0.f;
-        }
-      }
-      if constexpr (IO == IO_NCHW_BF16) {
-        fence_proxy_async_smem();
-        bar_sync(5, NUM_WORKERS);
-        if (threadIdx.x == WORKER_T0) {
-          __nv_bfloat16* gdst = static_cast<__nv_bfloat16*>(a.out) + size_t(tile) * spt * n_tok * D;
-          bulk_store_1d(gdst, smem + OFF_OUTST, uint32_t(seqs_here) * n_tok * D * 2);
-        }
+#pragma unroll
+          for (int j = 0; j < 32; j += 4) {
+            const float4 w4 = __ldg(reinterpret_cast<const float4*>(wl + c0 + j));
+            dot = fmaf(x[j], w4.x, fmaf(x[j + 1], w4.y, fmaf(x[j + 2], w4.z, fmaf(x[j + 3], w4.w, dot))));
+          }
+        }
+      }
+      if (logits) {
+        const float lg = w.exchange_sum(dot);
+        const size_t clip = grow / 12;
+        if (valid && g == 0) {
+          if (a.out21 != nullptr) a.out21[clip * 21 + t_in_seq] = lg;
+          if (a.decisions != nullptr) a.decisions[clip * 12 + t_in_seq] = lg > 0.f ? 1 : 0;
+        }
+        if (valid && g == 1 && t_in_seq < 9 && a.out21 != nullptr) a.out21[clip * 21 + 12 + t_in_seq] = 0.f;
       }
     }
     pf.mark(PW_OUTPUT);
     pf.count(PW_TILES);
   }
   pf.flush(0, 32);
-  if constexpr (IO == IO_NCHW_BF16) {
-    if (threadIdx.x == WORKER_T0) bulk_wait_all0();
+}
+
+template <int IO, int NTOK>
+__device__ void drain_main(const FusedArgs& a, uint64_t* bars, uint32_t tmem) {
+  const int q = (threadIdx.x >> 5) & 3, lane = threadIdx.x & 31, row = q * 32 + lane;
+  const uint32_t tl = tmem + (uint32_t(q * 32) << 16);
+  const int n_tok = NTOK ? NTOK : a.n_tok, slot = NTOK ? slot_of(NTOK) : a.slot, spt = NTOK ? 128 / slot_of(NTOK) : a.spt;
+  const int slot_log2 = NTOK ? log2_of(slot_of(NTOK)) : a.slot_log2;
+  const int seq_in_tile = row >> slot_log2, t_in_seq = row & (slot - 1);
+  for (uint32_t tk = 0;; ++tk) {
+    const int tile = next_tile(bars, tk);
+    if (tile < 0) break;
+    const TileTmem<IO> tm(tk);
+    const bool valid = seq_in_tile < min(spt, a.n_seq - tile * spt) && t_in_seq < n_tok;
+    __nv_bfloat16* dst = static_cast<__nv_bfloat16*>(a.out) + (size_t(tile) * spt + seq_in_tile) * n_tok * DIM + t_in_seq;
+    bar_wait(&bars[B_X_DONE], tk & 1u);
+    tc_fence_after();
+#pragma unroll 1
+    for (int c0 = 0; c0 < DIM; c0 += 32) {
+      float x[32];
+      tmem_ld32(tl + tm.x + c0, reinterpret_cast<uint32_t(&)[32]>(x));
+      tmem_ld_wait();
+      if (c0 + 32 == DIM) {
+        tc_fence_before();
+        __syncwarp();
+        if (lane == 0) mbar_arrive(&bars[B_DRAINED]);
+      }
+      if (valid) {
+#pragma unroll
+        for (int j = 0; j < 32; ++j) dst[(c0 + j) * n_tok] = __float2bfloat16_rn(x[j]);
+      }
+    }
   }
 }
 
 template <int IO, int D>
 __device__ void producer_main(const FusedArgs& a, uint8_t* smem, uint64_t* bars) {
-  uint32_t it = 0;
   int load_tile = blockIdx.x;
   uint32_t n_free = 0;
   bool need_free = false;
@@ -622,15 +653,7 @@
     const long long t0 = clock64();
     while (!mbar_try_wait(bar, parity)) {
       poll_loader();
-      if (clock64() - t0 > 4000000000LL) {
-        unsigned* tb = g_trap_buffer;
-        if (tb != nullptr) {
-          tb[0] = blockIdx.x; tb[1] = threadIdx.x; tb[2] = (smem_u32(bar) & 1023u) >> 3; tb[3] = parity;
-          __threadfence_system();
-        }
-        printf("avf: fused encoder producer timed out (block %d item %u)\n", blockIdx.x, it);
-        __trap();
-      }
+      if (clock64() - t0 > 4000000000LL) trap_timed_out(bar, parity);
     }
   };
   uint32_t gidx = 0;
@@ -639,7 +662,6 @@
     pbits ^= 1u << s;
     if (expect_bytes != 0) mbar_expect_tx(full_bar, expect_bytes);
     tma_load_2d(smem + slot_offset(s), tm, full_bar, c0, c1);
-    ++it;
   };
   uint32_t kpub = 0;
   auto publish = [&](int t) {
@@ -656,6 +678,9 @@
     if (nxt >= a.n_tiles) nxt = -1;
     publish(nxt);
     if (IO == IO_NCHW_BF16) {
+      if (nxt >= 0)
+        bulk_prefetch_l2(static_cast<const __nv_bfloat16*>(a.in) + size_t(nxt) * a.spt * a.n_tok * D,
+                         uint32_t(min(a.spt, a.n_seq - nxt * a.spt)) * a.n_tok * D * 2);
       while (load_tile >= 0) poll_loader();
       load_tile = nxt;
     }
@@ -695,19 +720,18 @@
 
 template <int IO, int D>
 __device__ void qkv_producer_main(const FusedArgs& a, uint8_t* smem, uint64_t* bars) {
-  uint32_t qit = 0, hq = 0, n_free = 0, n_read = 0;
+  uint32_t qit = 0, hq = 0, n_free = 0;
   bool first = true;
   for (uint32_t tk = 0; next_tile(bars, tk) >= 0; ++tk) {
-    if constexpr (IO == IO_NCHW_BF16) mbar_wait(&bars[B_OUT_READ], (n_read++) & 1);
     for (int l = 0; l < a.depth; ++l) {
       const LayerArgs& L = a.layer[l];
-      if (!first) mbar_wait(&bars[B_A1_FREE], (n_free++) & 1);
+      if (!first) bar_wait(&bars[B_A1_FREE], (n_free++) & 1);
       first = false;
       for (int h = 0; h < HEADS; ++h, ++hq) {
         uint64_t* fb = &bars[B_QG_FULL + (hq % uint32_t(NQG<D>))];
         for (int kp = 0; kp < KPH<D>; ++kp) {
           const uint32_t s = qit % QRING, ph = (qit / QRING) & 1;
-          mbar_wait(&bars[B_QR_EMPTY + s], ph ^ 1);
+          bar_wait(&bars[B_QR_EMPTY + s], ph ^ 1);
           uint8_t* d = smem + OFF_QRING + s * QSLOT_BYTES;
           if (kp == 0) mbar_expect_tx(fb, KPH<D> * QSLOT_BYTES);
           for (int s3 = 0; s3 < 3; ++s3) tma_load_2d(d + s3 * 4096, &L.tm_qkv, fb, kpanel<D>(kp) * 64, s3 * (HEADS * DH) + h * DH);
@@ -718,7 +742,7 @@
   }
 }
 
-template <int D>
+template <int IO, int D>
 __device__ void mma_main(const FusedArgs& a, uint8_t* smem, uint64_t* bars, uint32_t tmem) {
   const bool leader = elect_one();
   const uint32_t a0 = smem_u32(smem + OFF_A0);
@@ -728,12 +752,13 @@
   const uint32_t id_qkv = make_idesc_bf16(128, 96), id_s = make_idesc_bf16(128, kmax), id_pv = make_idesc_bf16(128, DH, 0, 1),
                  id_128 = make_idesc_bf16(128, 128), id_out = make_idesc_bf16(128, D);
   uint32_t obits = 0, m = 0, qit = 0, hq = 0, gidx = 0, n_a0 = 0, n_hready[2] = {0, 0};
+  uint32_t tx = 0, ts = 0;
   Prof pf;
   pf.start(blockIdx.x == 0 && leader);
   int ring_phase = PM_QKV;
   auto slot_wait = [&](uint32_t s) -> uint32_t {
     pf.mark(ring_phase);
-    mbar_wait(&bars[B_RING_FULL + s], (obits >> s) & 1u);
+    bar_wait(&bars[B_RING_FULL + s], (obits >> s) & 1u);
     obits ^= 1u << s;
     tc_fence_after();
     pf.mark(PM_RW_OUT);
@@ -741,7 +766,7 @@
   };
   auto group_wait = [&]() {
     pf.mark(ring_phase);
-    mbar_wait(&bars[B_G_FULL + (gidx & 7u)], (gidx >> 3) & 1u);
+    bar_wait(&bars[B_G_FULL + (gidx & 7u)], (gidx >> 3) & 1u);
     ++gidx;
     tc_fence_after();
     pf.mark(ring_phase == PM_FF1 ? PM_RW_FF1 : PM_RW_FF2);
@@ -753,19 +778,19 @@
     if constexpr (A0_HALF<D>) {
       if (!fresh || (i != 0 && i != 2)) return;
       pf.mark(ring_phase);
-      if (i == 0) mbar_wait(&bars[B_A0_HALF], n_a0 & 1);
-      else mbar_wait(&bars[B_A0_READY], (n_a0++) & 1);
+      if (i == 0) bar_wait(&bars[B_A0_HALF], n_a0 & 1);
+      else bar_wait(&bars[B_A0_READY], (n_a0++) & 1);
     } else {
       if (!fresh || i != 0) return;
       pf.mark(ring_phase);
-      mbar_wait(&bars[B_A0_READY], (n_a0++) & 1);
+      bar_wait(&bars[B_A0_READY], (n_a0++) & 1);
     }
     tc_fence_after();
     pf.mark(ring_phase == PM_QKV ? PM_WAIT_A0 : PM_WAIT_A0B);
   };
   auto qkv = [&](bool fresh) {
     pf.mark(ring_phase);
-    mbar_wait(&bars[B_QG_FULL + (hq % uint32_t(NQG<D>))], (hq / uint32_t(NQG<D>)) & 1u);
+    bar_wait(&bars[B_QG_FULL + (hq % uint32_t(NQG<D>))], (hq / uint32_t(NQG<D>)) & 1u);
     ++hq;
     tc_fence_after();
     pf.mark(PM_RW_QKV);
@@ -775,7 +800,7 @@
       const uint32_t s = qit % QRING;
       const uint64_t da = make_desc_sw128_kmajor(a0 + kp * 16384), db = make_desc_sw128_kmajor(qring + s * QSLOT_BYTES);
 #pragma unroll
-      for (int k = 0; k < 4; ++k) if (leader) umma_bf16(tmem + TM_D1, da + uint64_t(k * 2), db + uint64_t(k * 2), id_qkv, (i | k) != 0 ? 1u : 0u);
+      for (int k = 0; k < 4; ++k) if (leader) umma_bf16(ts + TM_D1, da + uint64_t(k * 2), db + uint64_t(k * 2), id_qkv, (i | k) != 0 ? 1u : 0u);
       if (leader) umma_commit(&bars[B_QR_EMPTY + s]);
       ++qit;
     }
@@ -784,13 +809,13 @@
   auto outproj = [&](int h) {
     const uint32_t s = RING_LO + h % (RING_HI - RING_LO), sb = slot_wait(s);
     const uint64_t db = desc_sw64(sb);
-    if (leader) umma_bf16_ts(tmem + TM_X, tmem + TM_O, db, id_out, 1u);
-    if (leader) umma_bf16_ts(tmem + TM_X, tmem + TM_O + 16, db + 2, id_out, 1u);
+    if (leader) umma_bf16_ts(tx, ts + TM_O, db, id_out, 1u);
+    if (leader) umma_bf16_ts(tx, ts + TM_O + 16, db + 2, id_out, 1u);
     slot_release(s);
   };
   bool last_layer = false;
   auto ff1 = [&](int c, bool fresh) {
-    const uint32_t d = tmem + ((c & 1) ? TM_H1 : TM_H0);
+    const uint32_t d = ts + ((c & 1) ? TM_H1 : TM_H0);
     for (int i = 0; i < D / 64; ++i) {
       const int kp = kpanel<D>(i);
       if (i % GSLOTS<D> == 0) group_wait();
@@ -806,26 +831,34 @@
   };
 
   for (uint32_t tk = 0; next_tile(bars, tk) >= 0; ++tk) {
+    const TileTmem<IO> tm(tk);
+    tx = tmem + tm.x;
+    ts = tmem + tm.s;
+    if (PINGPONG<IO> && tk > 0) {
+      bar_wait(&bars[B_DRAINED], (tk - 1) & 1u);
+      tc_fence_after();
+      pf.mark(PM_WAIT_DRAIN);
+    }
     for (int l = 0; l < a.depth; ++l) {
       last_layer = l == a.depth - 1;
       ring_phase = PM_QKV;
       qkv(true);
       pf.mark(PM_QKV);
       for (int h = 0; h < HEADS; ++h) {
-        mbar_wait(&bars[B_STAGED], h & 1);
+        bar_wait(&bars[B_STAGED], h & 1);
         tc_fence_after();
         pf.mark(PM_WAIT_STAGED);
         {
           const uint64_t da = desc_sw64(qs), db = desc_sw64(ks);
-          if (leader) umma_bf16(tmem + TM_S, da, db, id_s, 0u);
-          if (leader) umma_bf16(tmem + TM_S, da + 2, db + 2, id_s, 1u);
+          if (leader) umma_bf16(ts + TM_S, da, db, id_s, 0u);
+          if (leader) umma_bf16(ts + TM_S, da + 2, db + 2, id_s, 1u);
           if (leader) umma_commit(&bars[B_S_FULL]);
         }
         pf.mark(PM_S);
         if (h + 1 < HEADS) qkv(false);
         pf.mark(PM_QKV);
         if (h > 0) {
-          mbar_wait(&bars[B_O_DRAINED], (h - 1) & 1);
+          bar_wait(&bars[B_O_DRAINED], (h - 1) & 1);
           tc_fence_after();
           pf.mark(PM_WAIT_OD7);
           ring_phase = PM_OUT;
@@ -833,15 +866,15 @@
           pf.mark(PM_OUT);
           ring_phase = PM_QKV;
         }
-        mbar_wait(&bars[B_P_READY], h & 1);
+        bar_wait(&bars[B_P_READY], h & 1);
         tc_fence_after();
         pf.mark(PM_WAIT_P);
         for (int k = 0; k < kmax / 16; ++k)
-          if (leader) umma_bf16_ts(tmem + TM_O, tmem + TM_S + uint32_t(k * 8), desc_sw64(vs + (h & 1) * 8192 + k * 1024), id_pv, k != 0 ? 1u : 0u);
+          if (leader) umma_bf16_ts(ts + TM_O, ts + TM_S + uint32_t(k * 8), desc_sw64(vs + (h & 1) * 8192 + k * 1024), id_pv, k != 0 ? 1u : 0u);
         if (leader) umma_commit(&bars[B_O_FULL]);
         pf.mark(PM_PV);
       }
-      mbar_wait(&bars[B_O_DRAINED], (HEADS - 1) & 1);
+      bar_wait(&bars[B_O_DRAINED], (HEADS - 1) & 1);
       tc_fence_after();
       pf.mark(PM_WAIT_OD7);
       ring_phase = PM_OUT;
@@ -857,7 +890,7 @@
       for (int c = 0; c < a.n_chunks; ++c) {
         const int b = c & 1;
         pf.mark(PM_FF1);
-        mbar_wait(&bars[B_H_READY + b], (n_hready[b]++) & 1);
+        bar_wait(&bars[B_H_READY + b], (n_hready[b]++) & 1);
         tc_fence_after();
         pf.mark(PM_WAIT_H);
         ring_phase = PM_FF2;
@@ -865,10 +898,10 @@
           for (int nh = 0; nh < D / 128; ++nh) {
             if ((kp * (D / 128) + nh) % GSLOTS<D> == 0) group_wait();
             const uint32_t s = (m++) % RING, sb = smem0 + uint32_t(slot_offset(s));
-            const uint32_t ta = tmem + (b ? TM_H1 : TM_H0) + uint32_t(kp * 64);
+            const uint32_t ta = ts + (b ? TM_H1 : TM_H0) + uint32_t(kp * 64);
             const uint64_t db = make_desc_sw128_kmajor(sb);
 #pragma unroll
-            for (int k = 0; k < 4; ++k) if (leader) umma_bf16_ts(tmem + TM_X + nh * 128, ta + uint32_t(k * 8), db + uint64_t(k * 2), id_128, 1u);
+            for (int k = 0; k < 4; ++k) if (leader) umma_bf16_ts(tx + nh * 128, ta + uint32_t(k * 8), db + uint64_t(k * 2), id_128, 1u);
             slot_release(s);
           }
         pf.mark(PM_FF2);
@@ -876,6 +909,7 @@
         if (c + 2 < a.n_chunks) ff1(c + 2, false);
       }
       if (leader) umma_commit(&bars[B_X2_FULL]);
+      if (PINGPONG<IO> && last_layer && leader) umma_commit(&bars[B_X_DONE]);
       if (leader) umma_commit(&bars[B_A1_FREE]);
     }
   }
@@ -883,7 +917,7 @@
 }
 
 template <int IO, int NTOK, int D>
-__global__ void __launch_bounds__(NUM_THREADS, 1) encoder_fused_kernel(const __grid_constant__ FusedArgs a) {
+__global__ void __launch_bounds__(NUM_THREADS<IO>, 1) encoder_fused_kernel(const __grid_constant__ FusedArgs a) {
   extern __shared__ __align__(1024) uint8_t smem_raw[];
   uint8_t* smem = smem_raw;
   if (threadIdx.x == 0 && (smem_u32(smem_raw) & 1023u) != 0u) {
@@ -903,7 +937,7 @@
     }
     for (int i = 0; i < NUM_BARS; ++i) {
       const bool by_workers = i == B_A0_READY || i == B_A0_HALF || i == B_STAGED || i == B_P_READY || i == B_O_DRAINED || i == B_H_READY || i == B_H_READY1;
-      mbar_init(&bars[i], by_workers ? NUM_WORKERS / 32 : 1);
+      mbar_init(&bars[i], by_workers ? NUM_WORKERS / 32 : (i == B_DRAINED ? 4 : 1));
     }
     fence_barrier_init();
   }
@@ -918,14 +952,20 @@
   pdl_wait();
   pdl_trigger();
 
-  if (warp == 0) {
-    if (lane == 0) producer_main<IO, D>(a, smem, bars);
-  } else if (warp == 1) {
-    mma_main<D>(a, smem, bars, tmem);
-  } else if (warp == 2) {
-    if (lane == 0) qkv_producer_main<IO, D>(a, smem, bars);
+  if (threadIdx.x >= WORKER_T0<IO> && threadIdx.x < WORKER_T0<IO> + NUM_WORKERS) {
+    if constexpr (PINGPONG<IO>) asm volatile("setmaxnreg.inc.sync.aligned.u32 %0;" ::"n"(REG_WORKER));
+    worker_main<IO, NTOK, D>(a, smem, bars, tmem);
   } else {
-    worker_main<IO, NTOK, D>(a, smem, bars, tmem);
+    if constexpr (PINGPONG<IO>) asm volatile("setmaxnreg.dec.sync.aligned.u32 %0;" ::"n"(REG_SMALL));
+    if (warp == 0) {
+      if (lane == 0) producer_main<IO, D>(a, smem, bars);
+    } else if (warp == 1) {
+      mma_main<IO, D>(a, smem, bars, tmem);
+    } else if (warp == 2) {
+      if (lane == 0) qkv_producer_main<IO, D>(a, smem, bars);
+    } else if (PINGPONG<IO> && threadIdx.x >= WORKER_T0<IO> + NUM_WORKERS) {
+      drain_main<IO, NTOK>(a, bars, tmem);
+    }
   }
 
   tc_fence_before();
@@ -1020,13 +1060,13 @@
   const int cap = sm_cap();
   const int grid = min(a.n_tiles, cap > 0 ? min(cap, sm_count_cached()) : sm_count_cached());
   if (io_kind == IO_NCHW_BF16 && a.n_tok == 49)
-    launch_pdl(encoder_fused_kernel<IO_NCHW_BF16, 49, 256>, grid, NUM_THREADS, SMEM_ALLOC, st, a);
+    launch_pdl(encoder_fused_kernel<IO_NCHW_BF16, 49, 256>, grid, NUM_THREADS<IO_NCHW_BF16>, SMEM_ALLOC, st, a);
   else if (io_kind == IO_NCHW_BF16)
-    launch_pdl(encoder_fused_kernel<IO_NCHW_BF16, 0, 256>, grid, NUM_THREADS, SMEM_ALLOC, st, a);
+    launch_pdl(encoder_fused_kernel<IO_NCHW_BF16, 0, 256>, grid, NUM_THREADS<IO_NCHW_BF16>, SMEM_ALLOC, st, a);
   else if (D == 256)
-    launch_pdl(encoder_fused_kernel<IO_ROWS_F32, 0, 256>, grid, NUM_THREADS, SMEM_ALLOC, st, a);
+    launch_pdl(encoder_fused_kernel<IO_ROWS_F32, 0, 256>, grid, NUM_THREADS<IO_ROWS_F32>, SMEM_ALLOC, st, a);
   else
-    launch_pdl(encoder_fused_kernel<IO_ROWS_F32, 0, 128>, grid, NUM_THREADS, SMEM_ALLOC, st, a);
+    launch_pdl(encoder_fused_kernel<IO_ROWS_F32, 0, 128>, grid, NUM_THREADS<IO_ROWS_F32>, SMEM_ALLOC, st, a);
   AVF_LAUNCH_CHECK("encoder_fused_kernel");
   return 0;
 }
```

After: 498,500 (median of 6 runs). 1.02x the previous value.
